# diaoenmao/HeteroFL-Computation-and-Communication-Efficient-Federated-Learning-for-Heterogeneous-Clients

Measured on AMD Instinct MI355X. Metric: local-train samples/sec/node, higher is better.
Workload: dtype bfloat16; 1 GPU; model=resnet18, dataset=CIFAR10, control_name=1_100_0.1_iid_fix_a1-e1_bn_1_1, active_clients=10, local_epochs=5, global_batch=10, parallelism=client-dp1, engine=batched

## Files before the change

### heterofl_amd/fed/batched.py

```python
import math

import numpy as np
import torch
import torch.nn as nn
import torch.nn.functional as F

from .. import ops as native_ops


class BConv2d(nn.Module):

    def __init__(self, R, in_ch, out_ch, kernel, stride, padding, bias):
        super().__init__()
        self.R, self.in_ch, self.out_ch = R, in_ch, out_ch
        self.stride, self.padding = stride, padding
        self.weight = nn.Parameter(torch.empty(R * out_ch, in_ch, kernel, kernel))
        nn.init.kaiming_uniform_(self.weight, a=math.sqrt(5))
        if bias:
            bound = 1 / math.sqrt(in_ch * kernel * kernel)
            self.bias = nn.Parameter(torch.empty(R * out_ch).uniform_(-bound, bound))
        else:
            self.bias = None

    def forward(self, x, residual=None):
        if native_ops.use_native(x) and native_ops.native_conv_enabled():
            from ..ops.fused import grouped_conv
            return grouped_conv(x, self.weight, self.bias, self.R,
                                self.stride, self.padding, residual=residual)
        y = F.conv2d(x, self.weight, self.bias, stride=self.stride,
                     padding=self.padding, groups=self.R)
        return y if residual is None else y + residual


class BBatchNorm2d(nn.Module):

    def __init__(self, R, ch):
        super().__init__()
        self.weight = nn.Parameter(torch.ones(R * ch))
        self.bias = nn.Parameter(torch.zeros(R * ch))

    def forward(self, x):
        return F.batch_norm(x, None, None, self.weight, self.bias,
                            training=True, eps=1e-5)


class BGroupNorm(nn.Module):

    def __init__(self, R, groups, ch):
        super().__init__()
        self.num_groups = R * groups
        self.weight = nn.Parameter(torch.ones(R * ch))
        self.bias = nn.Parameter(torch.zeros(R * ch))

    def forward(self, x):
        return F.group_norm(x, self.num_groups, self.weight, self.bias, eps=1e-5)


class BLinear(nn.Module):

    def __init__(self, R, in_f, out_f):
        super().__init__()
        self.weight = nn.Parameter(torch.empty(R, out_f, in_f))
        nn.init.kaiming_uniform_(self.weight, a=math.sqrt(5))
        self.bias = nn.Parameter(torch.zeros(R, out_f))

    def forward(self, x):
        return torch.einsum('nri,roi->nro', x, self.weight) + self.bias


def batched_norm(norm, R, ch):
    if norm == 'bn':
        return BBatchNorm2d(R, ch)
    if norm == 'in':
        return BGroupNorm(R, ch, ch)
    if norm == 'ln':
        return BGroupNorm(R, 1, ch)
    if norm == 'gn':
        return BGroupNorm(R, 4, ch)
    if norm == 'none':
        return nn.Identity()
    raise ValueError('Not valid norm')


class BNormReLU(nn.Module):

    def __init__(self, R, ch, norm, rate, scale):
        super().__init__()
        self.norm = norm
        self.rate = rate if scale else 1.0
        self.stats_sink = None
        if norm == 'in':
            self.groups = R * ch
        elif norm == 'ln':
            self.groups = R
        elif norm == 'gn':
            self.groups = R * 4
        else:
            self.groups = 0
        if norm != 'none':
            self.weight = nn.Parameter(torch.ones(R * ch))
            self.bias = nn.Parameter(torch.zeros(R * ch))

    def forward(self, x):
        if self.norm == 'none':
            if self.training and self.rate != 1.0:
                if native_ops.use_native(x):
                    from ..ops.fused import fused_scaler
                    x = fused_scaler(x, self.rate)
                else:
                    x = x / self.rate
            return F.relu(x)
        kind = 'bn' if self.norm == 'bn' else 'gn'
        if native_ops.use_native(x):
            if self.stats_sink is not None and kind == 'bn':
                ext = native_ops.require_native()
                y, mean, invstd = ext.bn_relu_fwd(x.contiguous(), self.weight,
                                                  self.bias, 1e-5)
                self.stats_sink(self, mean, invstd, x)
                return y
            from ..ops.fused import fused_norm_relu
            return fused_norm_relu(x, self.weight, self.bias, kind,
                                   self.groups)
        if self.stats_sink is not None and kind == 'bn':
            mean = x.mean(dim=(0, 2, 3))
            var = x.var(dim=(0, 2, 3), unbiased=False)
            self.stats_sink(self, mean, (var + 1e-5).rsqrt(), x)
        from ..ops.fused import eager_scaler_norm_relu
        r = self.rate if self.training else 1.0
        return eager_scaler_norm_relu(x, self.weight, self.bias, kind,
                                      self.groups, r)


class BMaxPool2(nn.Module):

    def forward(self, x):
        if native_ops.use_native(x):
            from ..ops.fused import fused_maxpool2
            return fused_maxpool2(x)
        return F.max_pool2d(x, 2)


class BScaler(nn.Module):
    def __init__(self, rate):
        super().__init__()
        self.rate = rate

    def forward(self, x):
        if not self.training or self.rate == 1.0:
            return x
        if native_ops.use_native(x):
            from ..ops.fused import fused_scaler
            return fused_scaler(x, self.rate)
        return x / self.rate


class BBlock(nn.Module):
    expansion = 1

    def __init__(self, R, in_planes, planes, stride, rate, norm, scale):
        super().__init__()
        self.n1 = BNormReLU(R, in_planes, norm, rate, scale)
        self.conv1 = BConv2d(R, in_planes, planes, 3, stride, 1, bias=False)
        self.n2 = BNormReLU(R, planes, norm, rate, scale)
        self.conv2 = BConv2d(R, planes, planes, 3, 1, 1, bias=False)
        if stride != 1 or in_planes != self.expansion * planes:
            self.shortcut = BConv2d(R, in_planes, self.expansion * planes,
                                    1, stride, 0, bias=False)

    def forward(self, x):
        out = self.n1(x)
        shortcut = self.shortcut(out) if hasattr(self, 'shortcut') else x
        out = self.conv1(out)
        return self.conv2(self.n2(out), residual=shortcut)


class BBottleneck(nn.Module):
    expansion = 4

    def __init__(self, R, in_planes, planes, stride, rate, norm, scale):
        super().__init__()
        self.n1 = BNormReLU(R, in_planes, norm, rate, scale)
        self.conv1 = BConv2d(R, in_planes, planes, 1, 1, 0, bias=False)
        self.n2 = BNormReLU(R, planes, norm, rate, scale)
        self.conv2 = BConv2d(R, planes, planes, 3, stride, 1, bias=False)
        self.n3 = BNormReLU(R, planes, norm, rate, scale)
        self.conv3 = BConv2d(R, planes, self.expansion * planes, 1, 1, 0,
                             bias=False)
        if stride != 1 or in_planes != self.expansion * planes:
            self.shortcut = BConv2d(R, in_planes, self.expansion * planes,
                                    1, stride, 0, bias=False)

    def forward(self, x):
        out = self.n1(x)
        shortcut = self.shortcut(out) if hasattr(self, 'shortcut') else x
        out = self.conv1(out)
        out = self.conv2(self.n2(out))
        return self.conv3(self.n3(out), residual=shortcut)


class BatchedResNet(nn.Module):

    def __init__(self, R, data_shape, hidden_size, num_blocks, num_classes,
                 rate, norm, scale, block=BBlock):
        super().__init__()
        self.R = R
        self.num_classes = num_classes
        self.data_ch = data_shape[0]
        self.in_planes = hidden_size[0]
        self.conv1 = BConv2d(R, data_shape[0], hidden_size[0], 3, 1, 1, bias=False)
        self.layer1 = self._make_layer(R, block, hidden_size[0], num_blocks[0], 1, rate, norm, scale)
        self.layer2 = self._make_layer(R, block, hidden_size[1], num_blocks[1], 2, rate, norm, scale)
        self.layer3 = self._make_layer(R, block, hidden_size[2], num_blocks[2], 2, rate, norm, scale)
        self.layer4 = self._make_layer(R, block, hidden_size[3], num_blocks[3], 2, rate, norm, scale)
        self.n4 = BNormReLU(R, hidden_size[3] * block.expansion, norm, rate, scale)
        self.linear = BLinear(R, hidden_size[3] * block.expansion, num_classes)

    def _make_layer(self, R, block, planes, num_blocks, stride, rate, norm, scale):
        strides = [stride] + [1] * (num_blocks - 1)
        layers = []
        for s in strides:
            layers.append(block(R, self.in_planes, planes, s, rate, norm, scale))
            self.in_planes = planes * block.expansion
        return nn.Sequential(*layers)

    def forward(self, x):
        out = self.conv1(x)
        out = self.layer1(out)
        out = self.layer2(out)
        out = self.layer3(out)
        out = self.layer4(out)
        out = self.n4(out)
        if native_ops.use_native(out):
            from ..ops.fused import fused_head
            return fused_head(out, self.linear.weight, self.linear.bias,
                              self.R)
        out = F.adaptive_avg_pool2d(out, 1)
        out = out.view(out.size(0), self.R, -1)
        return self.linear(out)


class BatchedConv(nn.Module):

    def __init__(self, R, data_shape, hidden_size, num_classes, rate, norm, scale):
        super().__init__()
        self.R = R
        self.num_classes = num_classes
        blocks = []
        in_ch = data_shape[0]
        for i, out_ch in enumerate(hidden_size):
            blocks.append(BConv2d(R, in_ch, out_ch, 3, 1, 1, bias=True))
            blocks.append(nn.Identity())
            blocks.append(BNormReLU(R, out_ch, norm, rate, scale))
            blocks.append(nn.Identity())
            if i != len(hidden_size) - 1:
                blocks.append(BMaxPool2())
            in_ch = out_ch
        self.blocks = nn.Sequential(*blocks)
        self._feat = hidden_size[-1]
        self.head = BLinear(R, hidden_size[-1], num_classes)

    def forward(self, x):
        out = self.blocks(x)
        if native_ops.use_native(out):
            from ..ops.fused import fused_head
            return fused_head(out, self.head.weight, self.head.bias, self.R)
        out = F.adaptive_avg_pool2d(out, 1).view(out.size(0), self.R, -1)
        return self.head(out)


def pack_states(batched, locals_list):
    R = batched.R
    bsd = batched.state_dict()
    key_map = _key_map(batched, locals_list[0])
    with torch.no_grad():
        for bk, lk in key_map.items():
            bt = bsd[bk]
            vals = [locals_list[r][lk] for r in range(R)]
            if bt.dim() == 3:
                src = torch.stack(vals, 0)
            elif bt.dim() == 2:
                src = torch.stack(vals, 0)
            else:
                src = torch.cat(vals, 0)
            bt.copy_(src.to(bt.device, bt.dtype))


def unpack_states(batched, template_keys):
    R = batched.R
    bsd = batched.state_dict()
    key_map = _key_map_from_keys(batched, template_keys)
    outs = [dict() for _ in range(R)]
    for bk, lk in key_map.items():
        bt = bsd[bk].detach()
        if bt.dim() in (2, 3):
            for r in range(R):
                outs[r][lk] = bt[r].clone()
        else:
            per = bt.size(0) // R
            for r in range(R):
                outs[r][lk] = bt[r * per:(r + 1) * per].clone()
    return outs


def _key_map(batched, local_sd):
    return _key_map_from_keys(batched, list(local_sd.keys()))


def _key_map_from_keys(batched, local_keys):
    bkeys = list(batched.state_dict().keys())
    if isinstance(batched, BatchedConv):
        lin_w = [k for k in local_keys if 'weight' in k][-1]
        lin_b = [k for k in local_keys if 'bias' in k][-1]
        m = {}
        for bk in bkeys:
            if bk == 'head.weight':
                m[bk] = lin_w
            elif bk == 'head.bias':
                m[bk] = lin_b
            else:
                m[bk] = bk
        return m
    return {bk: bk for bk in bkeys}


def batched_masked_ce(scores, labels, label_masks, metrics=None):
    if native_ops.use_native(scores):
        from ..ops.fused import fused_masked_ce
        return fused_masked_ce(scores, labels, label_masks, metrics)
    N, R, C = scores.shape
    if label_masks is not None:
        scores = scores.masked_fill(label_masks.unsqueeze(0) == 0, 0)
    logp = F.log_softmax(scores, dim=2)
    nll = -logp.gather(2, labels.unsqueeze(2)).squeeze(2)
    losses = nll.mean(0)
    if metrics is not None:
        with torch.no_grad():
            correct = (scores.argmax(2) == labels).float().sum(0)
            metrics[:, 0] += losses.detach() * N
            metrics[:, 1] += correct
            metrics[:, 2] += N
    return losses


def per_client_clip_(params, R, max_norm=1.0):
    sq = None
    views = []
    for p in params:
        if p.grad is None:
            continue
        g = p.grad
        if g.size(0) % R != 0:
            raise RuntimeError(f'grad shape {tuple(g.shape)} not divisible by R={R}')
        v = g.view(R, -1)
        views.append((g, v))
        s = (v.float() ** 2).sum(dim=1)
        sq = s if sq is None else sq + s
    if sq is None:
        return None
    total = sq.sqrt()
    scale = (max_norm / (total + 1e-6)).clamp(max=1.0)
    for g, v in views:
        v.mul_(scale.unsqueeze(1).to(v.dtype))
    return total


class DeviceAugment:

    def __init__(self, data_name, device):
        self.data_name = data_name
        if data_name in ('MNIST', 'FashionMNIST'):
            mean, std = (0.1307,), (0.3081,)
            self.crop = False
        else:
            mean, std = (0.4914, 0.4822, 0.4465), (0.2023, 0.1994, 0.2010)
            self.crop = True
        self.mean = torch.tensor(mean, device=device).view(1, -1, 1, 1)
        self.std = torch.tensor(std, device=device).view(1, -1, 1, 1)

    def __call__(self, img_u8, train=True):
        x = img_u8.permute(0, 3, 1, 2).float().div_(255.0)
        n, C, H, W = x.shape
        if train and self.crop:
            pad = 4
            xp = F.pad(x, [pad] * 4)
            dy = torch.randint(0, 2 * pad + 1, (n,), device=x.device)
            dx = torch.randint(0, 2 * pad + 1, (n,), device=x.device)
            rows = dy.view(n, 1) + torch.arange(H, device=x.device).view(1, H)
            idx_r = rows.view(n, 1, H, 1).expand(n, C, H, W + 2 * pad)
            xp = xp.gather(2, idx_r)
            cols = dx.view(n, 1) + torch.arange(W, device=x.device).view(1, W)
            idx_c = cols.view(n, 1, 1, W).expand(n, C, H, W)
            x = xp.gather(3, idx_c)
            flip = torch.rand(n, device=x.device) < 0.5
            x = torch.where(flip.view(n, 1, 1, 1), x.flip(-1), x)
        return (x - self.mean) / self.std


class BatchedClientTrainer:

    def __init__(self, cfg):
        self.cfg = cfg
        self.device = torch.device(cfg['device'])
        self.dataset = None
        self.data_split = None
        self.augment = None
        self._amp = (cfg.get('compute_dtype') in ('bfloat16', 'fp8')
                     and self.device.type == 'cuda')
        if self.device.type == 'cuda':
            native_ops.set_fp8(cfg.get('compute_dtype') == 'fp8')
        self._shard_cache = {}
        self._model_cache = {}
        self._graph_cache = {}

    def set_data(self, dataset, data_split):
        self.dataset = dataset['train']
        self.data_split = data_split['train']
        self.augment = DeviceAugment(self.cfg['data_name'], self.device)
        self._shard_cache.clear()

    def _shard(self, user):
        if user not in self._shard_cache:
            idx = torch.tensor(self.data_split[user], dtype=torch.long)
            img = self.dataset.img[idx]
            if img.dim() == 3:
                img = img.unsqueeze(-1)
            labels = torch.tensor([self.dataset.target[i] for i in idx.tolist()],
                                  dtype=torch.long)
            self._shard_cache[user] = (img.to(self.device, non_blocking=True),
                                       labels.to(self.device, non_blocking=True))
        return self._shard_cache[user]

    def _batched_model(self, rate, R, scaler_rate=None):
        key = (rate, R) if scaler_rate is None else (rate, R, scaler_rate)
        if key not in self._model_cache:
            cfg = self.cfg
            name = cfg['model_name']
            if scaler_rate is None:
                scaler_rate = rate / cfg['global_model_rate']
            if 'resnet' in name:
                hidden = [int(np.ceil(rate * h)) for h in cfg['resnet']['hidden_size']]
                nb, blk = {'resnet18': ([2, 2, 2, 2], BBlock),
                           'resnet34': ([3, 4, 6, 3], BBlock),
                           'resnet50': ([3, 4, 6, 3], BBottleneck),
                           'resnet101': ([3, 4, 23, 3], BBottleneck),
                           'resnet152': ([3, 8, 36, 3], BBottleneck)}[name]
                model = BatchedResNet(R, cfg['data_shape'], hidden, nb,
                                      cfg['classes_size'], scaler_rate,
                                      cfg['norm'], cfg['scale'], block=blk)
            elif name == 'conv':
                hidden = [int(np.ceil(rate * h)) for h in cfg['conv']['hidden_size']]
                model = BatchedConv(R, cfg['data_shape'], hidden,
                                    cfg['classes_size'], scaler_rate,
                                    cfg['norm'], cfg['scale'])
            else:
                raise NotImplementedError(name)
            self._model_cache[key] = model.to(self.device)
        return self._model_cache[key]

    def train_clients(self, client_slots, user_idx, local_parameters,
                      model_rate, make_loader, label_split, lr, logger=None):
        if self.dataset is None:
            raise RuntimeError('BatchedClientTrainer.set_data was not called')
        cfg = self.cfg
        B = cfg['batch_size']['train']
        groups = {}
        for m in client_slots:
            u = user_idx[m]
            n = len(self.data_split[u])
            sched = tuple([B] * (n // B) + ([n % B] if n % B else []))
            groups.setdefault((model_rate[u], sched), []).append(m)
        out = []
        import os as _os
        gsplit = int(_os.environ.get('HETEROFL_GROUP_SPLIT', '1'))
        split_groups = {}
        for (rate, sched), slots in groups.items():
            if gsplit > 1 and self.device.type == 'cuda' \
                    and len(slots) >= 2 * gsplit:
                per = (len(slots) + gsplit - 1) // gsplit
                for si in range(0, len(slots), per):
                    split_groups[(rate, sched, si)] = slots[si:si + per]
            else:
                split_groups[(rate, sched, 0)] = slots
        graphed = []
        for (rate, sched, tag), slots in split_groups.items():
            use_graph = (self.device.type == 'cuda'
                         and cfg.get('hip_graphs', True)
                         and len(set(sched)) == 1)
            if use_graph:
                graphed.append((rate, sched, slots, tag))
            else:
                out.extend(self._train_group(rate, sched, slots, user_idx,
                                             local_parameters, label_split,
                                             lr, logger))
        if graphed:
            preps = [self._prepare_graphed(rate, sched, slots, user_idx,
                                           [local_parameters[m]
                                            for m in slots],
                                           label_split, lr, tag)
                     for rate, sched, slots, tag in graphed]
            from .runner import _phase_timer
            with _phase_timer('2d.replay'):
                if len(preps) > 1:
                    if not hasattr(self, '_streams') or \
                            len(self._streams) < len(preps):
                        self._streams = [torch.cuda.Stream()
                                         for _ in range(len(preps))]
                    cur = torch.cuda.current_stream()
                    events = []
                    for (gs, x_cat, y_cat, nspe), st in zip(preps,
                                                            self._streams):
                        st.wait_stream(cur)
                        with torch.cuda.stream(st):
                            gs.run_epochs(x_cat, y_cat, nspe)
                        ev = torch.cuda.Event()
                        ev.record(st)
                        events.append(ev)
                    for ev in events:
                        cur.wait_event(ev)
                else:
                    gs, x_cat, y_cat, nspe = preps[0]
                    gs.run_epochs(x_cat, y_cat, nspe)
            for (rate, sched, slots, tag), (gs, _, _, _) in zip(graphed,
                                                                preps):
                out.extend(self._finish_graphed(
                    gs, slots, [local_parameters[m] for m in slots], logger))
        return out

    def _graph_step(self, rate, sched, R, lr, tag=0):
        from .graphs import GraphedGroupStep
        key = (rate, R, tuple(sched), lr, tag)
        if key not in self._graph_cache:
            cfg = self.cfg
            model = self._batched_model(rate, R)
            self._model_cache.pop((rate, R), None)
            model.train(True)
            capacity = sum(sched) * cfg['num_epochs']['local']
            self._graph_cache[key] = GraphedGroupStep(
                model, R, sched[0], lr, cfg['momentum'], cfg['weight_decay'],
                cfg['classes_size'], capacity, self._amp, self.device)
        return self._graph_cache[key]

    def _train_group(self, rate, sched, slots, user_idx, local_parameters,
                     label_split, lr, logger=None):
        cfg = self.cfg
        R = len(slots)
        device = self.device
        use_graph = (device.type == 'cuda' and cfg.get('hip_graphs', True)
                     and len(set(sched)) == 1)
        locals_list = [local_parameters[m] for m in slots]
        if use_graph:
            return self._train_group_graphed(rate, sched, slots, user_idx,
                                             locals_list, label_split, lr,
                                             logger)
        model = self._batched_model(rate, R)
        pack_states(model, locals_list)
        model.train(True)
        params = [p for p in model.parameters() if p.requires_grad]
        native = native_ops.use_native(device)
        if native:
            if not hasattr(self, '_opt_cache'):
                self._opt_cache = {}
            cached = self._opt_cache.get((rate, R))
            if cached is None or cached[0] is not model:
                from ..ops.fused import FusedClipSGD
                for p in params:
                    p.grad = torch.zeros_like(p)
                bufs = [torch.zeros_like(p) for p in params]
                cached = (model, FusedClipSGD(params,
                                              [p.grad for p in params],
                                              bufs, R, device))
                self._opt_cache[(rate, R)] = cached
            fopt = cached[1]
            for b in fopt.bufs:
                b.zero_()
            opt = None
        else:
            opt = torch.optim.SGD(params, lr=lr, momentum=cfg['momentum'],
                                  weight_decay=cfg['weight_decay'])
        masks = None
        if cfg['mask']:
            masks = torch.zeros(R, cfg['classes_size'], device=device)
            for i, m in enumerate(slots):
                masks[i, label_split[user_idx[m]]] = 1
        shards = [self._shard(user_idx[m]) for m in slots]
        n = sum(sched)
        for _ in range(cfg['num_epochs']['local']):
            xs, ys = [], []
            for img, lab in shards:
                perm = torch.randperm(img.size(0), device=device)
                xs.append(self.augment(img[perm], train=True))
                ys.append(lab[perm])
            x_all = torch.stack(xs, 1)
            x_all = x_all.reshape(n, -1, x_all.size(-2), x_all.size(-1))
            if self._amp:
                x_all = x_all.to(torch.bfloat16)
            y_all = torch.stack(ys, 1)
            off = 0
            for bs in sched:
                xb = x_all[off:off + bs]
                yb = y_all[off:off + bs]
                off += bs
                if native:
                    torch._foreach_zero_([p.grad for p in params])
                else:
                    opt.zero_grad(set_to_none=True)
                with torch.autocast('cuda', torch.bfloat16, enabled=self._amp):
                    scores = model(xb)
                losses = batched_masked_ce(scores.float(), yb, masks)
                losses.sum().backward()
                if native:
                    fopt.step(1.0, lr, cfg['momentum'], cfg['weight_decay'])
                else:
                    per_client_clip_(params, R, 1.0)
                    opt.step()
                if logger is not None:
                    with torch.no_grad():
                        sc = scores
                        if masks is not None:
                            sc = sc.masked_fill(masks.unsqueeze(0) == 0, 0)
                        pred = sc.argmax(dim=2)
                        acc = (pred == yb).float().mean(0) * 100.0
                        for i in range(R):
                            logger.append({'Local-Loss': losses[i].item(),
                                           'Local-Accuracy': acc[i].item()},
                                          'train', n=bs)
        template_keys = list(locals_list[0].keys())
        states = unpack_states(model, template_keys)
        cpu_or_dev = [{k: v for k, v in st.items()} for st in states]
        return list(zip(slots, cpu_or_dev))

    def _prepare_graphed(self, rate, sched, slots, user_idx, locals_list,
                         label_split, lr, tag=0):
        from .runner import _phase_timer
        cfg = self.cfg
        R = len(slots)
        device = self.device
        with _phase_timer('2a.graph_build'):
            gs = self._graph_step(rate, sched, R, lr, tag)
            if gs.graph is None:
                gs.ensure_captured()
        with _phase_timer('2b.pack'):
            pack_states(gs.model, locals_list)
        masks = None
        if cfg['mask']:
            masks = torch.zeros(R, cfg['classes_size'], device=device)
            for i, m in enumerate(slots):
                masks[i, label_split[user_idx[m]]] = 1
        gs.begin_round(masks)
        shards = [self._shard(user_idx[m]) for m in slots]
        n = sum(sched)
        E = cfg['num_epochs']['local']
        with _phase_timer('2c.stage_augment'):
            xs_ep, ys_ep = [], []
            for _ in range(E):
                xs, ys = [], []
                for img, lab in shards:
                    perm = torch.randperm(img.size(0), device=device)
                    xs.append(self.augment(img[perm], train=True))
                    ys.append(lab[perm])
                x_all = torch.stack(xs, 1)
                xs_ep.append(x_all.reshape(n, -1, x_all.size(-2), x_all.size(-1)))
                ys_ep.append(torch.stack(ys, 1))
            x_cat = torch.cat(xs_ep, 0)
            if self._amp:
                x_cat = x_cat.to(torch.bfloat16)
            y_cat = torch.cat(ys_ep, 0)
        return gs, x_cat, y_cat, len(sched)

    def _finish_graphed(self, gs, slots, locals_list, logger=None):
        from .runner import _phase_timer
        R = len(slots)
        if logger is not None:
            m = gs.metrics.detach().cpu()
            for i in range(R):
                cnt = max(int(m[i, 2].item()), 1)
                logger.append({'Local-Loss': m[i, 0].item() / cnt,
                               'Local-Accuracy': m[i, 1].item() / cnt * 100.0},
                              'train', n=cnt)
        with _phase_timer('2e.unpack'):
            template_keys = list(locals_list[0].keys())
            states = unpack_states(gs.model, template_keys)
        return list(zip(slots, [dict(st) for st in states]))
```

### heterofl_amd/fed/graphs.py

```python
import torch

from .. import ops as native_ops
from .batched import batched_masked_ce


class GraphedGroupStep:

    def __init__(self, model, R, batch, lr, momentum, weight_decay, classes,
                 capacity, amp, device):
        self.model = model
        self.R = R
        self.batch = batch
        self.lr = lr
        self.momentum = momentum
        self.weight_decay = weight_decay
        self.amp = amp
        self.device = device
        self.params = [p for p in model.parameters() if p.requires_grad]
        self.bufs = [torch.zeros_like(p) for p in self.params]
        self.capacity = capacity
        shape = self._input_shape()
        xdt = torch.bfloat16 if amp else torch.float32
        self.x_all = torch.zeros(capacity, *shape, device=device, dtype=xdt)
        self.y_all = torch.zeros(capacity, R, dtype=torch.long, device=device)
        self.masks = torch.ones(R, classes, device=device)
        self.counter = torch.zeros(1, dtype=torch.long, device=device)
        self.metrics = torch.zeros(R, 3, device=device)
        self.graph = None
        self._arange = torch.arange(batch, device=device)
        self._native = (device.type == 'cuda' and native_ops.use_native(device))
        self._capturing = False
        self._captured_grads = None
        self._shadows = False
        if self._native:
            native_ops.require_native()
            from ..ops.fused import GraphClipSGD
            self.opt = GraphClipSGD(self.params, self.bufs, R, device)

    def _input_shape(self):
        m = self.model
        w = next(p for p in m.parameters() if p.dim() == 4)
        in_ch = w.size(1)
        hw = 32 if in_ch == 3 else 28
        return (self.R * in_ch, hw, hw)

    def _one_step(self):
        idx = self.counter * self.batch + self._arange
        xb = self.x_all.index_select(0, idx)
        yb = self.y_all.index_select(0, idx)
        if self._native:
            with torch.autocast('cuda', torch.bfloat16, enabled=self.amp):
                scores = self.model(xb)
            losses = batched_masked_ce(scores.float(), yb, self.masks,
                                       metrics=self.metrics)
            raw = torch.autograd.grad(losses.sum(), self.params)
            grads = [t if t.is_contiguous() else t.contiguous() for t in raw]
            self._captured_grads = grads
            if not self._capturing:
                self.opt.bind(grads)
            self.opt.launch(1.0, self.lr, self.momentum, self.weight_decay)
            with torch.no_grad():
                self.counter += 1
            return
        with torch.autocast('cuda', torch.bfloat16, enabled=self.amp):
            scores = self.model(xb)
            losses = batched_masked_ce(scores.float(), yb, self.masks)
        loss = losses.sum()
        raw = torch.autograd.grad(loss, self.params)
        with torch.no_grad():
            grads = [g.contiguous() for g in raw]
            sq = None
            views = [g.view(self.R, -1) for g in grads]
            for v in views:
                s = (v.float() ** 2).sum(dim=1)
                sq = s if sq is None else sq + s
            scale = (1.0 / (sq.sqrt() + 1e-6)).clamp(max=1.0)
            for v in views:
                v.mul_(scale.unsqueeze(1).to(v.dtype))
            torch._foreach_add_(grads, self.params, alpha=self.weight_decay)
            torch._foreach_mul_(self.bufs, self.momentum)
            torch._foreach_add_(self.bufs, grads)
            torch._foreach_add_(self.params, self.bufs, alpha=-self.lr)
            pred = scores.argmax(dim=2)
            correct = (pred == yb).float().sum(0)
            self.metrics[:, 0] += losses.detach() * self.batch
            self.metrics[:, 1] += correct
            self.metrics[:, 2] += self.batch
            self.counter += 1

    def capture(self):
        saved_p = [p.detach().clone() for p in self.params]
        saved_b = [b.clone() for b in self.bufs]
        saved_m = self.metrics.clone()
        torch.cuda.synchronize()
        s = torch.cuda.Stream()
        s.wait_stream(torch.cuda.current_stream())
        with torch.cuda.stream(s):
            for _ in range(3):
                self.counter.zero_()
                self._one_step()
        torch.cuda.current_stream().wait_stream(s)
        self.counter.zero_()
        self.graph = torch.cuda.CUDAGraph()
        self._capturing = True
        with torch.cuda.graph(self.graph):
            self._one_step()
        self._capturing = False
        if self._native:
            self.opt.bind(self._captured_grads)
        with torch.no_grad():
            for p, sp in zip(self.params, saved_p):
                p.copy_(sp)
            for b, sb in zip(self.bufs, saved_b):
                b.copy_(sb)
            self.metrics.copy_(saved_m)
            self.counter.zero_()
        if self._shadows:
            from .batched_lm import refresh_shadows
            refresh_shadows(self.model)
        torch.cuda.synchronize()

    def begin_round(self, masks):
        with torch.no_grad():
            if masks is not None:
                self.masks.copy_(masks)
            else:
                self.masks.fill_(1)
            for b in self.bufs:
                b.zero_()
            self.metrics.zero_()

    def run_epochs(self, x_epochs, y_epochs, steps_per_epoch):
        total = x_epochs.size(0)
        with torch.no_grad():
            self.x_all[:total].copy_(x_epochs)
            self.y_all[:total].copy_(y_epochs)
            self.counter.zero_()
        n_steps = total // self.batch
        if self.graph is None:
            self.capture()
        for _ in range(n_steps):
            self.graph.replay()

    def ensure_captured(self):
        if self.graph is None:
            self.capture()


class LMGraphedStep:

    def __init__(self, model, R, n_rows, bptt, n_win, lr, momentum,
                 weight_decay, num_tokens, amp, device):
        self.model = model
        self.R = R
        self.bptt = bptt
        self.n_win = n_win
        self.lr = lr
        self.momentum = momentum
        self.weight_decay = weight_decay
        self.amp = amp
        self.device = device
        self.params = [p for p in model.parameters() if p.requires_grad]
        self.bufs = [torch.zeros_like(p) for p in self.params]
        self.windows = torch.zeros(n_win, R, n_rows, bptt, dtype=torch.long,
                                   device=device)
        self.masks = torch.ones(R, num_tokens, device=device)
        self.counter = torch.zeros(1, dtype=torch.long, device=device)
        self.metrics = torch.zeros(R, 3, device=device)
        self.graph = None
        self._capturing = False
        self._captured_grads = None
        self._native = (device.type == 'cuda' and native_ops.use_native(device))
        smap = getattr(model, '_shadow_map', None) or {}
        self._shadows = bool(smap)
        if self._native:
            from ..ops.fused import GraphClipSGD
            self.opt = GraphClipSGD(self.params, self.bufs, R, device,
                                    shadows=[smap.get(id(p))
                                             for p in self.params]
                                    if smap else None)

    def _one_step(self):
        w = self.counter - (self.counter // self.n_win) * self.n_win
        tokens = self.windows.index_select(0, w).squeeze(0)
        self._step_on(tokens)
        with torch.no_grad():
            self.counter += 1

    def tail_step(self, tokens):
        self._step_on(tokens)
        if self._native and self.graph is not None:
            self.opt.bind(self._graph_grads)

    def _step_on(self, tokens):
        from .batched_lm import lm_masked_ce
        with torch.autocast('cuda', torch.bfloat16,
                            enabled=self.amp and not self._shadows):
            logits = self.model(tokens)
        losses = lm_masked_ce(logits, tokens, self.masks)
        with torch.no_grad():
            n = tokens.size(1)
            ld = losses.detach()
            self.metrics[:, 0] += ld * n
            self.metrics[:, 1] += torch.exp(ld.clamp(max=30.0)) * n
            self.metrics[:, 2] += n
        if self._native:
            raw = torch.autograd.grad(losses.sum(), self.params)
            grads = [t if t.is_contiguous() else t.contiguous() for t in raw]
            self._captured_grads = grads
            if not self._capturing:
                self.opt.bind(grads)
            self.opt.launch(1.0, self.lr, self.momentum, self.weight_decay)
            if self._shadows:
                from ..ops.fused import bump_rng
                bump_rng(self.device)
        else:
            raw = torch.autograd.grad(losses.sum(), self.params)
            with torch.no_grad():
                grads = [g.contiguous() for g in raw]
                sq = None
                views = [g.view(self.R, -1) for g in grads]
                for v in views:
                    s = (v.float() ** 2).sum(dim=1)
                    sq = s if sq is None else sq + s
                scale = (1.0 / (sq.sqrt() + 1e-6)).clamp(max=1.0)
                for v in views:
                    v.mul_(scale.unsqueeze(1).to(v.dtype))
                torch._foreach_add_(grads, self.params,
                                    alpha=self.weight_decay)
                torch._foreach_mul_(self.bufs, self.momentum)
                torch._foreach_add_(self.bufs, grads)
                torch._foreach_add_(self.params, self.bufs, alpha=-self.lr)

    def capture(self):
        saved_p = [p.detach().clone() for p in self.params]
        saved_b = [b.clone() for b in self.bufs]
        saved_m = self.metrics.clone()
        torch.cuda.synchronize()
        s = torch.cuda.Stream()
        s.wait_stream(torch.cuda.current_stream())
        with torch.cuda.stream(s):
            for _ in range(3):
                self.counter.zero_()
                self._one_step()
        torch.cuda.current_stream().wait_stream(s)
        self.counter.zero_()
        self.graph = torch.cuda.CUDAGraph()
        self._capturing = True
        with torch.cuda.graph(self.graph):
            self._one_step()
        self._capturing = False
        if self._native:
            self._graph_grads = self._captured_grads
            self.opt.bind(self._graph_grads)
        with torch.no_grad():
            for p, sp in zip(self.params, saved_p):
                p.copy_(sp)
            for b, sb in zip(self.bufs, saved_b):
                b.copy_(sb)
            self.metrics.copy_(saved_m)
            self.counter.zero_()
        if self._shadows:
            from .batched_lm import refresh_shadows
            refresh_shadows(self.model)
        torch.cuda.synchronize()

    def begin_round(self, rows, masks):
        with torch.no_grad():
            for w in range(self.n_win):
                self.windows[w].copy_(
                    rows[:, :, w * self.bptt:(w + 1) * self.bptt])
            if masks is not None:
                self.masks.copy_(masks)
            else:
                self.masks.fill_(1)
            for b in self.bufs:
                b.zero_()
            self.metrics.zero_()
            self.counter.zero_()

    def run_window_pass(self):
        if self.graph is None:
            self.capture()
        for _ in range(self.n_win):
            self.graph.replay()
```

### heterofl_amd/ops/__init__.py

```python
import os

import torch

_ext = None
_ext_err = None


def _load():
    global _ext, _ext_err
    if _ext is not None or _ext_err is not None:
        return _ext
    try:
        from . import _heterofl_hip as ext
        _ext = ext
    except ImportError as e:
        _ext_err = e
    return _ext


def native_available():
    return _load() is not None


def require_native():
    if os.environ.get('HETEROFL_FORCE_EAGER') == '1':
        return None
    ext = _load()
    if ext is None:
        raise RuntimeError(
            f'heterofl_amd native HIP extension is not built '
            f'(import error: {_ext_err}). Build it with '
            f'`python setup.py build_ext --inplace` (PYTORCH_ROCM_ARCH=gfx950).')
    return ext


def use_native(tensor_or_device=None):
    if os.environ.get('HETEROFL_FORCE_EAGER') == '1':
        return False
    if isinstance(tensor_or_device, torch.Tensor):
        is_cuda = tensor_or_device.is_cuda
    elif tensor_or_device is not None:
        is_cuda = torch.device(tensor_or_device).type == 'cuda'
    else:
        is_cuda = torch.cuda.is_available()
    return is_cuda


def native_conv_enabled():
    return os.environ.get('HETEROFL_NATIVE_CONV', '1') == '1'


_FP8 = False


def set_fp8(on):
    global _FP8
    _FP8 = bool(on)


def fp8_enabled():
    return _FP8


_LARGE_CONV = os.environ.get('HETEROFL_LARGE_CONV', '0') == '1'


def set_large_conv(on):
    global _LARGE_CONV
    prev = _LARGE_CONV
    _LARGE_CONV = bool(on)
    return prev


def large_conv_enabled():
    return _LARGE_CONV
```

### heterofl_amd/ops/csrc/bindings.cpp

```cpp
#include <torch/extension.h>

std::vector<at::Tensor> bn_relu_fwd(at::Tensor x, at::Tensor gamma,
                                    at::Tensor beta, double eps);
std::vector<at::Tensor> bn_relu_bwd(at::Tensor dy, at::Tensor x,
                                    at::Tensor gamma, at::Tensor beta,
                                    at::Tensor mean, at::Tensor invstd);
std::string bn_relu_route(const std::string& direction, int64_t N, int64_t C,
                          int64_t HW, int64_t elem_size, bool aligned);
std::vector<at::Tensor> gn_relu_fwd(at::Tensor x, at::Tensor gamma,
                                    at::Tensor beta, int64_t G, double eps);
std::vector<at::Tensor> gn_relu_bwd(at::Tensor dy, at::Tensor x,
                                    at::Tensor gamma, at::Tensor beta,
                                    at::Tensor mean, at::Tensor invstd,
                                    int64_t G);
std::vector<at::Tensor> masked_ce_fwd(at::Tensor scores, at::Tensor labels,
                                      at::Tensor mask, at::Tensor metrics);
at::Tensor masked_ce_bwd(at::Tensor scores, at::Tensor labels, at::Tensor mask,
                         at::Tensor up);
std::vector<at::Tensor> build_chunk_table(std::vector<at::Tensor> grads,
                                          std::vector<at::Tensor> params,
                                          std::vector<at::Tensor> bufs,
                                          int64_t R, int64_t chunk_elems,
                                          std::vector<at::Tensor> shadows);
void fill_chunk_table(at::Tensor blob, std::vector<at::Tensor> grads,
                      std::vector<at::Tensor> params,
                      std::vector<at::Tensor> bufs, int64_t R,
                      int64_t chunk_elems, std::vector<at::Tensor> shadows);
void clip_sgd_step(at::Tensor table_blob, int64_t n_chunks,
                   at::Tensor chunk_client, at::Tensor partials,
                   at::Tensor normsq, double max_norm, double lr,
                   double momentum, double weight_decay);
at::Tensor conv_fwd(at::Tensor x, at::Tensor w, at::Tensor bias,
                    at::Tensor residual, int64_t groups, int64_t stride,
                    int64_t pad, int64_t fp8);
at::Tensor conv_bwd_data(at::Tensor dy, at::Tensor w, int64_t groups,
                         int64_t stride, int64_t pad, int64_t H, int64_t W,
                         int64_t fp8);
at::Tensor conv_bwd_weight(at::Tensor dy, at::Tensor x, int64_t groups,
                           int64_t stride, int64_t pad, int64_t khw,
                           int64_t fp8);
std::tuple<std::string, int64_t, int64_t> conv_plan(
    const std::string& direction, int64_t G, int64_t N, int64_t Cin,
    int64_t H, int64_t W, int64_t Cout, int64_t khw, int64_t stride,
    int64_t pad, int64_t elem_size, int64_t fp8);
std::string conv_plan_variant(
    const std::string& direction, int64_t G, int64_t N, int64_t Cin,
    int64_t H, int64_t W, int64_t Cout, int64_t khw, int64_t stride,
    int64_t pad, int64_t elem_size, int64_t fp8);
at::Tensor mfma_probe(at::Tensor A, at::Tensor B);
std::vector<at::Tensor> head_fwd(at::Tensor feat, at::Tensor w, at::Tensor b,
                                 int64_t R);
std::vector<at::Tensor> attn_fwd(at::Tensor q, at::Tensor k, at::Tensor v,
                                 double temperature);
std::vector<at::Tensor> attn_bwd(at::Tensor dout, at::Tensor q, at::Tensor k,
                                 at::Tensor v, at::Tensor p,
                                 double temperature);
std::vector<at::Tensor> attn_fwd_block(at::Tensor q, at::Tensor k,
                                       at::Tensor v, double temperature);
std::vector<at::Tensor> attn_bwd_block(at::Tensor dout, at::Tensor q,
                                       at::Tensor k, at::Tensor v,
                                       at::Tensor out, at::Tensor lse,
                                       double temperature);
std::vector<at::Tensor> ln_fwd(at::Tensor x, at::Tensor gamma,
                               at::Tensor beta, int64_t R, double eps);
std::vector<at::Tensor> ln_bwd(at::Tensor dy, at::Tensor x, at::Tensor gamma,
                               at::Tensor mean, at::Tensor invstd, int64_t R);
std::vector<at::Tensor> lm_ce_fwd(at::Tensor logits, at::Tensor labels,
                                  at::Tensor mask, int64_t R);
at::Tensor lm_ce_bwd(at::Tensor logits, at::Tensor labels, at::Tensor mask,
                     at::Tensor row_max, at::Tensor row_logsum,
                     at::Tensor up, int64_t R);
std::vector<at::Tensor> head_bwd(at::Tensor dscores, at::Tensor pooled,
                                 at::Tensor w, int64_t R, int64_t H,
                                 int64_t W, bool bf16_feat, bool want_db);
void rng_bump(at::Tensor seed);
std::vector<at::Tensor> gelu_drop_fwd(at::Tensor x, at::Tensor seed,
                                      int64_t salt, double rate, double p);
at::Tensor gelu_drop_bwd(at::Tensor dy, at::Tensor x, at::Tensor mask,
                         double rate, double p);
std::vector<at::Tensor> res_drop_fwd(at::Tensor src, at::Tensor h,
                                     at::Tensor seed, int64_t salt,
                                     double rate, double p);
at::Tensor drop_scale_bwd(at::Tensor dt, at::Tensor mask, double rate,
                          double p);
at::Tensor token_mask(at::Tensor tokens, at::Tensor seed, int64_t salt,
                      double rate, int64_t mask_id);
at::Tensor embed_pos_fwd(at::Tensor ids, at::Tensor table, at::Tensor pos,
                         double rate);
std::vector<at::Tensor> embed_pos_bwd(at::Tensor dy, at::Tensor ids,
                                      int64_t V, int64_t P, double rate);
std::vector<at::Tensor> maxpool2_fwd(at::Tensor x);
void pack_slices(at::Tensor blob, int64_t n, int64_t max_rows);
void pack_slices_roll(at::Tensor spans, int64_t n_spans, at::Tensor blocks);
void combine_accumulate(at::Tensor table, int64_t n_tensors,
                        int64_t n_entries, at::Tensor blocks);
at::Tensor maxpool2_bwd(at::Tensor dy, at::Tensor arg, int64_t H,
                        int64_t W);
at::Tensor conv_pack_weight(at::Tensor w);
at::Tensor conv_fwd_large(at::Tensor x, at::Tensor packed, at::Tensor bias,
                          at::Tensor residual, int64_t stride, int64_t pad,
                          int64_t Cin, int64_t Cout, int64_t k);
at::Tensor bn_relu_infer(at::Tensor x, at::Tensor scale, at::Tensor shift);
std::vector<at::Tensor> eval_metrics(at::Tensor scores, at::Tensor labels,
                                     at::Tensor user_ptr,
                                     at::Tensor user_samples,
                                     at::Tensor label_mask);
at::Tensor lm_head_pack(at::Tensor w);
std::vector<at::Tensor> lm_head_ce(at::Tensor x, at::Tensor packed,
                                   at::Tensor bias, at::Tensor labels,
                                   at::Tensor vocab_mask, int64_t V,
                                   int64_t E, int64_t splits);
std::vector<at::Tensor> lm_head_topk(at::Tensor x, at::Tensor packed,
                                     at::Tensor bias, at::Tensor labels,
                                     at::Tensor vocab_mask, int64_t V,
                                     int64_t E, int64_t k, int64_t splits);
int64_t lm_head_topk_splits(int64_t M, int64_t V);

PYBIND11_MODULE(TORCH_EXTENSION_NAME, m) {
    m.def("bn_relu_fwd", &bn_relu_fwd, "fused sBN+ReLU forward");
    m.def("bn_relu_bwd", &bn_relu_bwd, "fused sBN+ReLU backward");
    m.def("bn_relu_route", &bn_relu_route,
          "name of the kernel route bn_relu_fwd / bn_relu_bwd would take; "
          "launches nothing");
    m.def("gn_relu_fwd", &gn_relu_fwd, "fused GroupNorm+ReLU forward");
    m.def("gn_relu_bwd", &gn_relu_bwd, "fused GroupNorm+ReLU backward");
    m.def("masked_ce_fwd", &masked_ce_fwd, "batched masked CE forward");
    m.def("masked_ce_bwd", &masked_ce_bwd, "batched masked CE backward");
    m.def("build_chunk_table", &build_chunk_table,
          "build clip+SGD chunk table");
    m.def("clip_sgd_step", &clip_sgd_step, "fused per-client clip+SGD step");
    m.def("fill_chunk_table", &fill_chunk_table,
          "fill a preallocated chunk table post-capture");
    m.def("conv_fwd", &conv_fwd, "MFMA implicit-GEMM grouped conv forward");
    m.def("conv_bwd_data", &conv_bwd_data, "MFMA grouped conv backward-data");
    m.def("conv_bwd_weight", &conv_bwd_weight,
          "MFMA grouped conv backward-weight (fp32 out)");
    m.def("conv_plan", &conv_plan,
          "(route, split, dynamic LDS bytes) the conv launchers would take; "
          "launches nothing");
    m.def("conv_plan_variant", &conv_plan_variant,
          "name of the kernel the conv launcher would launch; launches "
          "nothing");
    m.def("mfma_probe", &mfma_probe, "16x16x32 bf16 MFMA layout probe");
    m.def("head_fwd", &head_fwd, "fused avgpool+per-client-linear forward");
    m.def("head_bwd", &head_bwd, "fused head backward");
    m.def("attn_fwd", &attn_fwd, "fused small-S attention forward");
    m.def("attn_bwd", &attn_bwd, "fused small-S attention backward");
    m.def("attn_fwd_block", &attn_fwd_block,
          "blockwise (flash-style) attention forward, any S");
    m.def("attn_bwd_block", &attn_bwd_block,
          "blockwise attention backward (deterministic two-pass)");
    m.def("ln_fwd", &ln_fwd, "fused per-client LayerNorm forward");
    m.def("ln_bwd", &ln_bwd, "fused per-client LayerNorm backward");
    m.def("lm_ce_fwd", &lm_ce_fwd, "fused vocab-masked LM CE forward");
    m.def("lm_ce_bwd", &lm_ce_bwd, "fused vocab-masked LM CE backward");
    m.def("rng_bump", &rng_bump, "advance the device RNG seed cell");
    m.def("gelu_drop_fwd", &gelu_drop_fwd, "fused scaler+GELU+dropout fwd");
    m.def("gelu_drop_bwd", &gelu_drop_bwd, "fused scaler+GELU+dropout bwd");
    m.def("res_drop_fwd", &res_drop_fwd,
          "fused scaler+dropout+residual-add fwd");
    m.def("drop_scale_bwd", &drop_scale_bwd,
          "dropout-mask * 1/rate backward");
    m.def("token_mask", &token_mask, "Bernoulli token masking (in-kernel RNG)");
    m.def("embed_pos_fwd", &embed_pos_fwd,
          "fused token+positional embedding gather with Scaler");
    m.def("embed_pos_bwd", &embed_pos_bwd,
          "deterministic embedding backward (fp32 master grads)");
    m.def("maxpool2_fwd", &maxpool2_fwd, "2x2/2 MaxPool forward (saves argmax)");
    m.def("pack_slices", &pack_slices,
          "one-launch distribute slice pack from a descriptor table");
    m.def("pack_slices_roll", &pack_slices_roll,
          "one-launch distribute pack of periodic-window (rolled / per-head) "
          "slices");
    m.def("combine_accumulate", &combine_accumulate,
          "one-launch deterministic combine accumulator + count (gather "
          "form)");
    m.def("maxpool2_bwd", &maxpool2_bwd, "2x2/2 MaxPool backward");
    m.def("conv_pack_weight", &conv_pack_weight,
          "one-time tap-major bf16 repack for conv_fwd_large");
    m.def("conv_fwd_large", &conv_fwd_large,
          "large-batch forward conv (bf16, groups=1, packed weight)");
    m.def("bn_relu_infer", &bn_relu_infer,
          "eval-mode BN+ReLU from folded scale/shift");
    m.def("eval_metrics", &eval_metrics,
          "per-user Local + Global evaluation sums (deterministic)");
    m.def("lm_head_pack", &lm_head_pack,
          "one-time padded bf16 repack of the LM vocabulary head");
    m.def("lm_head_ce", &lm_head_ce,
          "fused vocabulary projection + cross-entropy (no logits written)");
    m.def("lm_head_topk", &lm_head_topk,
          "fused vocabulary projection + top-k + log-sum-exp (no logits "
          "written)");
    m.def("lm_head_topk_splits", &lm_head_topk_splits,
          "lm_head_topk's own choice of splits for M rows");
}
```

### heterofl_amd/ops/csrc/fused_norm.hip

```cpp
#include "common.h"

template <typename T, bool STAGE>
__global__ void __launch_bounds__(256)
bn_relu_fwd_kernel(const T* __restrict__ x, const float* __restrict__ gamma,
                   const float* __restrict__ beta, T* __restrict__ y,
                   float* __restrict__ mean_out, float* __restrict__ invstd_out,
                   int N, int C, int HW, float eps) {
    const int c = blockIdx.x;
    __shared__ float scratch[2 * 256 / WAVE];
    extern __shared__ __attribute__((aligned(16))) char smem[];
    T* stage = (T*)smem;
    float s1 = 0.f, s2 = 0.f;
    const long chan_off = (long)c * HW;
    const long samp_stride = (long)C * HW;
    for (int i = threadIdx.x; i < N * HW; i += blockDim.x) {
        const int n = i / HW, hw = i - n * HW;
        const T raw = x[n * samp_stride + chan_off + hw];
        if (STAGE) stage[i] = raw;
        const float v = (float)raw;
        s1 += v;
        s2 += v * v;
    }
    block_reduce2(s1, s2, scratch);
    const float inv_m = 1.f / (N * HW);
    const float mean = s1 * inv_m;
    const float var = fmaxf(s2 * inv_m - mean * mean, 0.f);
    const float invstd = rsqrtf(var + eps);
    if (threadIdx.x == 0) {
        mean_out[c] = mean;
        invstd_out[c] = invstd;
    }
    const float g = gamma ? gamma[c] : 1.f;
    const float b = beta ? beta[c] : 0.f;
    const float scale = invstd * g;
    const float shift = b - mean * scale;
    for (int i = threadIdx.x; i < N * HW; i += blockDim.x) {
        const int n = i / HW, hw = i - n * HW;
        const long off = n * samp_stride + chan_off + hw;
        const float v = STAGE ? (float)stage[i] : ld_f32(x + off);
        st_f32(y + off, fmaxf(v * scale + shift, 0.f));
    }
}

template <typename T>
__global__ void __launch_bounds__(256)
bn_sums_kernel(const T* __restrict__ x, float* __restrict__ partials, int N,
               int C, int HW, int S) {
    const int c = blockIdx.x;
    const int s = blockIdx.y;
    const int chunk = (N + S - 1) / S;
    const int n1 = min(N, (s + 1) * chunk);
    const long chan_off = (long)c * HW;
    const long samp_stride = (long)C * HW;
    float s1 = 0.f, s2 = 0.f;
    for (int n = s * chunk; n < n1; ++n) {
        const T* base = x + n * samp_stride + chan_off;
        for (int hw = threadIdx.x; hw < HW; hw += blockDim.x) {
            const float v = ld_f32(base + hw);
            s1 += v;
            s2 += v * v;
        }
    }
    __shared__ float scratch[2 * 256 / WAVE];
    block_reduce2(s1, s2, scratch);
    if (threadIdx.x == 0) {
        partials[((long)c * S + s) * 2] = s1;
        partials[((long)c * S + s) * 2 + 1] = s2;
    }
}

__global__ void __launch_bounds__(256)
bn_finalize_kernel(const float* __restrict__ partials,
                   const float* __restrict__ gamma,
                   const float* __restrict__ beta,
                   float* __restrict__ mean_out,
                   float* __restrict__ invstd_out,
                   float* __restrict__ scale_shift, int C, int S,
                   float inv_m, float eps) {
    const int c = blockIdx.x * blockDim.x + threadIdx.x;
    if (c >= C) return;
    float s1 = 0.f, s2 = 0.f;
    for (int s = 0; s < S; ++s) {
        s1 += partials[((long)c * S + s) * 2];
        s2 += partials[((long)c * S + s) * 2 + 1];
    }
    const float mean = s1 * inv_m;
    const float var = fmaxf(s2 * inv_m - mean * mean, 0.f);
    const float invstd = rsqrtf(var + eps);
    mean_out[c] = mean;
    invstd_out[c] = invstd;
    const float g = gamma ? gamma[c] : 1.f;
    const float b = beta ? beta[c] : 0.f;
    const float scale = invstd * g;
    scale_shift[2 * c] = scale;
    scale_shift[2 * c + 1] = b - mean * scale;
}

template <typename T>
__global__ void __launch_bounds__(256)
bn_apply_relu_kernel(const T* __restrict__ x,
                     const float* __restrict__ scale_shift,
                     T* __restrict__ y, int N, int C, int HW, int S) {
    const int c = blockIdx.x;
    const int s = blockIdx.y;
    const int chunk = (N + S - 1) / S;
    const int n1 = min(N, (s + 1) * chunk);
    const long chan_off = (long)c * HW;
    const long samp_stride = (long)C * HW;
    const float scale = scale_shift[2 * c];
    const float shift = scale_shift[2 * c + 1];
    for (int n = s * chunk; n < n1; ++n) {
        const long off = n * samp_stride + chan_off;
        for (int hw = threadIdx.x; hw < HW; hw += blockDim.x)
            st_f32(y + off + hw, fmaxf(ld_f32(x + off + hw) * scale + shift,
                                       0.f));
    }
}

template <typename T, bool STAGE>
__global__ void __launch_bounds__(256)
bn_relu_bwd_kernel(const T* __restrict__ dy, const T* __restrict__ x,
                   const float* __restrict__ gamma, const float* __restrict__ beta,
                   const float* __restrict__ mean, const float* __restrict__ invstd,
                   T* __restrict__ dx, float* __restrict__ dgamma,
                   float* __restrict__ dbeta, int N, int C, int HW) {
    const int c = blockIdx.x;
    __shared__ float scratch[2 * 256 / WAVE];
    extern __shared__ __attribute__((aligned(16))) char smem[];
    T* sx = (T*)smem;
    T* sd = sx + (STAGE ? N * HW : 0);
    const long chan_off = (long)c * HW;
    const long samp_stride = (long)C * HW;
    const float m = mean[c], is = invstd[c];
    const float g = gamma ? gamma[c] : 1.f;
    const float b = beta ? beta[c] : 0.f;
    float s1 = 0.f, s2 = 0.f;
    for (int i = threadIdx.x; i < N * HW; i += blockDim.x) {
        const int n = i / HW, hw = i - n * HW;
        const long off = n * samp_stride + chan_off + hw;
        const T xr = x[off];
        const float xh = ((float)xr - m) * is;
        const float pre = xh * g + b;
        const float d = pre > 0.f ? ld_f32(dy + off) : 0.f;
        if (STAGE) {
            sx[i] = xr;
            sd[i] = (T)d;
        }
        s1 += d;
        s2 += d * xh;
    }
    block_reduce2(s1, s2, scratch);
    if (threadIdx.x == 0) {
        dbeta[c] = s1;
        dgamma[c] = s2;
    }
    const float inv_M = 1.f / (N * HW);
    const float k1 = s1 * inv_M, k2 = s2 * inv_M;
    const float gis = g * is;
    for (int i = threadIdx.x; i < N * HW; i += blockDim.x) {
        const int n = i / HW, hw = i - n * HW;
        const long off = n * samp_stride + chan_off + hw;
        float xh, d;
        if (STAGE) {
            xh = ((float)sx[i] - m) * is;
            d = (float)sd[i];
        } else {
            xh = (ld_f32(x + off) - m) * is;
            const float pre = xh * g + b;
            d = pre > 0.f ? ld_f32(dy + off) : 0.f;
        }
        st_f32(dx + off, gis * (d - k1 - xh * k2));
    }
}

constexpr int BN_VEC_U = 4;

struct RowWalk {
    int n, j, dn, dj, vpr;
    __device__ __forceinline__ RowWalk(int v, int vpr_) : vpr(vpr_) {
        n = v / vpr;
        j = v - n * vpr;
        dn = 256 / vpr;
        dj = 256 - dn * vpr;
    }
    __device__ __forceinline__ void step() {
        j += dj;
        n += dn;
        if (j >= vpr) {
            j -= vpr;
            ++n;
        }
    }
};

template <typename T>
__global__ void __launch_bounds__(256)
bn_relu_fwd_vec_kernel(const T* __restrict__ x,
                       const float* __restrict__ gamma,
                       const float* __restrict__ beta, T* __restrict__ y,
                       float* __restrict__ mean_out,
                       float* __restrict__ invstd_out, int N, int C, int HW,
                       float eps) {
    constexpr int V = 16 / sizeof(T);
    const int c = blockIdx.x;
    __shared__ float scratch[2 * 256 / WAVE];
    extern __shared__ __attribute__((aligned(16))) char smem[];
    const T* stage = (const T*)smem;
    uint4* stage4 = (uint4*)smem;
    const int M = N * HW;
    const int nvec = M / V;
    const long samp_stride = (long)C * HW;
    const T* xc = x + (long)c * HW;
    T* yc = y + (long)c * HW;
    RowWalk rw(threadIdx.x, HW / V);
    for (int v0 = threadIdx.x; v0 < nvec; v0 += 256 * BN_VEC_U) {
        uint4 r[BN_VEC_U];
        const long off0 = rw.n * samp_stride + rw.j * V;
#pragma unroll
        for (int u = 0; u < BN_VEC_U; ++u) {
            const long off = v0 + u * 256 < nvec
                                 ? rw.n * samp_stride + rw.j * V : off0;
            r[u] = *(const uint4*)(xc + off);
            rw.step();
        }
#pragma unroll
        for (int u = 0; u < BN_VEC_U; ++u)
            if (v0 + u * 256 < nvec) stage4[v0 + u * 256] = r[u];
    }
    __syncthreads();
    float s1 = 0.f, s2 = 0.f;
#pragma unroll 8
    for (int i = threadIdx.x; i < M; i += 256) {
        const float v = (float)stage[i];
        s1 += v;
        s2 += v * v;
    }
    block_reduce2(s1, s2, scratch);
    const float inv_m = 1.f / (N * HW);
    const float mean = s1 * inv_m;
    const float var = fmaxf(s2 * inv_m - mean * mean, 0.f);
    const float invstd = rsqrtf(var + eps);
    if (threadIdx.x == 0) {
        mean_out[c] = mean;
        invstd_out[c] = invstd;
    }
    const float g = gamma ? gamma[c] : 1.f;
    const float b = beta ? beta[c] : 0.f;
    const float scale = invstd * g;
    const float shift = b - mean * scale;
    RowWalk ww(threadIdx.x, HW / V);
    for (int v = threadIdx.x; v < nvec; v += 256) {
        float f[V];
        unpack16<T>(stage4[v], f);
#pragma unroll
        for (int e = 0; e < V; ++e) f[e] = fmaxf(f[e] * scale + shift, 0.f);
        *(uint4*)(yc + ww.n * samp_stride + ww.j * V) = pack16<T>(f);
        ww.step();
    }
}

template <typename T>
__global__ void __launch_bounds__(256)
bn_relu_bwd_vec_kernel(const T* __restrict__ dy, const T* __restrict__ x,
                       const float* __restrict__ gamma,
                       const float* __restrict__ beta,
                       const float* __restrict__ mean,
                       const float* __restrict__ invstd, T* __restrict__ dx,
                       float* __restrict__ dgamma, float* __restrict__ dbeta,
                       int N, int C, int HW) {
    constexpr int V = 16 / sizeof(T);
    const int c = blockIdx.x;
    __shared__ float scratch[2 * 256 / WAVE];
    extern __shared__ __attribute__((aligned(16))) char smem[];
    const int M = N * HW;
    const int nvec = M / V;
    const T* sx = (const T*)smem;
    const T* sd = sx + M;
    uint4* sx4 = (uint4*)sx;
    uint4* sd4 = (uint4*)sd;
    const long samp_stride = (long)C * HW;
    const T* xc = x + (long)c * HW;
    const T* dyc = dy + (long)c * HW;
    T* dxc = dx + (long)c * HW;
    const float m = mean[c], is = invstd[c];
    const float g = gamma ? gamma[c] : 1.f;
    const float b = beta ? beta[c] : 0.f;
    RowWalk rw(threadIdx.x, HW / V);
    for (int v0 = threadIdx.x; v0 < nvec; v0 += 256 * BN_VEC_U) {
        uint4 rx[BN_VEC_U], rd[BN_VEC_U];
        const long off0 = rw.n * samp_stride + rw.j * V;
#pragma unroll
        for (int u = 0; u < BN_VEC_U; ++u) {
            const long off = v0 + u * 256 < nvec
                                 ? rw.n * samp_stride + rw.j * V : off0;
            rx[u] = *(const uint4*)(xc + off);
            rd[u] = *(const uint4*)(dyc + off);
            rw.step();
        }
#pragma unroll
        for (int u = 0; u < BN_VEC_U; ++u)
            if (v0 + u * 256 < nvec) {
                sx4[v0 + u * 256] = rx[u];
                sd4[v0 + u * 256] = rd[u];
            }
    }
    __syncthreads();
    float s1 = 0.f, s2 = 0.f;
#pragma unroll 8
    for (int i = threadIdx.x; i < M; i += 256) {
        const float xh = ((float)sx[i] - m) * is;
        const float pre = xh * g + b;
        const float d = pre > 0.f ? ld_f32(sd + i) : 0.f;
        s1 += d;
        s2 += d * xh;
    }
    block_reduce2(s1, s2, scratch);
    if (threadIdx.x == 0) {
        dbeta[c] = s1;
        dgamma[c] = s2;
    }
    const float inv_M = 1.f / (N * HW);
    const float k1 = s1 * inv_M, k2 = s2 * inv_M;
    const float gis = g * is;
    RowWalk ww(threadIdx.x, HW / V);
    for (int v = threadIdx.x; v < nvec; v += 256) {
        float fx[V], fd[V];
        unpack16<T>(sx4[v], fx);
        unpack16<T>(sd4[v], fd);
#pragma unroll
        for (int e = 0; e < V; ++e) {
            const float xh = (fx[e] - m) * is;
            const float pre = xh * g + b;
            const float d = pre > 0.f ? fd[e] : 0.f;
            fd[e] = gis * (d - k1 - xh * k2);
        }
        *(uint4*)(dxc + ww.n * samp_stride + ww.j * V) = pack16<T>(fd);
        ww.step();
    }
}

__device__ __forceinline__ float mul_rn(float a, float b) {
#pragma clang fp contract(off)
    return a * b;
}
__device__ __forceinline__ float sub_rn(float a, float b) {
#pragma clang fp contract(off)
    return a - b;
}

template <typename T, bool STAGE>
__global__ void __launch_bounds__(256)
gn_relu_fwd_kernel(const T* __restrict__ x, const float* __restrict__ gamma,
                   const float* __restrict__ beta, T* __restrict__ y,
                   float* __restrict__ mean_out, float* __restrict__ invstd_out,
                   int N, int C, int HW, int G, float eps) {
    const int ng = blockIdx.x;
    const int n = ng / G, j = ng - n * G;
    const int cpg = C / G;
    __shared__ float scratch[2 * 256 / WAVE];
    extern __shared__ __attribute__((aligned(16))) char smem[];
    T* stage = (T*)smem;
    const long base = (long)n * C * HW + (long)j * cpg * HW;
    const int M = cpg * HW;
    float s1 = 0.f, s2 = 0.f;
    for (int i = threadIdx.x; i < M; i += blockDim.x) {
        const T raw = x[base + i];
        if (STAGE) stage[i] = raw;
        const float v = (float)raw;
        s1 += v;
        s2 += v * v;
    }
    block_reduce2(s1, s2, scratch);
    const float inv_m = 1.f / M;
    const float mean = s1 * inv_m;
    const float var = fmaxf(sub_rn(mul_rn(s2, inv_m), mul_rn(mean, mean)),
                            0.f);
    const float invstd = rsqrtf(var + eps);
    if (threadIdx.x == 0) {
        mean_out[ng] = mean;
        invstd_out[ng] = invstd;
    }
    for (int i = threadIdx.x; i < M; i += blockDim.x) {
        const int c = j * cpg + i / HW;
        const float g = gamma ? gamma[c] : 1.f;
        const float b = beta ? beta[c] : 0.f;
        const float v = STAGE ? (float)stage[i] : ld_f32(x + base + i);
        st_f32(y + base + i, fmaxf((v - mean) * invstd * g + b, 0.f));
    }
}

template <typename T>
__global__ void __launch_bounds__(256)
gn_relu_bwd_kernel(const T* __restrict__ dy, const T* __restrict__ x,
                   const float* __restrict__ gamma, const float* __restrict__ beta,
                   const float* __restrict__ mean, const float* __restrict__ invstd,
                   T* __restrict__ dx, float* __restrict__ pgamma,
                   float* __restrict__ pbeta, int N, int C, int HW, int G) {
    const int ng = blockIdx.x;
    const int n = ng / G, j = ng - n * G;
    const int cpg = C / G;
    __shared__ float scratch[2 * 256 / WAVE];
    const long base = (long)n * C * HW + (long)j * cpg * HW;
    const int M = cpg * HW;
    const float m = mean[ng], is = invstd[ng];
    if (pgamma) {
        for (int cc = threadIdx.x; cc < cpg; cc += blockDim.x) {
            const int c = j * cpg + cc;
            const float g = gamma ? gamma[c] : 1.f;
            const float b = beta ? beta[c] : 0.f;
            float sg = 0.f, sb = 0.f;
            for (int hw = 0; hw < HW; ++hw) {
                const long off = base + (long)cc * HW + hw;
                const float xh = (ld_f32(x + off) - m) * is;
                const float pre = xh * g + b;
                const float d = pre > 0.f ? ld_f32(dy + off) : 0.f;
                sg += d * xh;
                sb += d;
            }
            pgamma[(long)n * C + c] = sg;
            pbeta[(long)n * C + c] = sb;
        }
    }
    float s1 = 0.f, s2 = 0.f;
    for (int i = threadIdx.x; i < M; i += blockDim.x) {
        const int c = j * cpg + i / HW;
        const float g = gamma ? gamma[c] : 1.f;
        const float b = beta ? beta[c] : 0.f;
        const float xh = (ld_f32(x + base + i) - m) * is;
        const float pre = xh * g + b;
        const float d = pre > 0.f ? ld_f32(dy + base + i) : 0.f;
        const float dg = mul_rn(d, g);
        s1 += dg;
        s2 += dg * xh;
    }
    block_reduce2(s1, s2, scratch);
    const float inv_M = 1.f / M;
    const float k1 = s1 * inv_M, k2 = s2 * inv_M;
    for (int i = threadIdx.x; i < M; i += blockDim.x) {
        const int c = j * cpg + i / HW;
        const float g = gamma ? gamma[c] : 1.f;
        const float b = beta ? beta[c] : 0.f;
        const float xh = (ld_f32(x + base + i) - m) * is;
        const float pre = xh * g + b;
        const float d = pre > 0.f ? ld_f32(dy + base + i) : 0.f;
        st_f32(dx + base + i,
               is * (sub_rn(mul_rn(d, g), k1) - xh * k2));
    }
}

#include <torch/extension.h>
#include <ATen/hip/HIPContext.h>

#define DISPATCH_FT(t, ...)                                                   \
    if ((t) == at::kFloat) { using scalar_t = float; __VA_ARGS__; }           \
    else if ((t) == at::kBFloat16) { using scalar_t = __hip_bfloat16; __VA_ARGS__; } \
    else { TORCH_CHECK(false, "unsupported dtype"); }

enum BnRoute { BN_VEC, BN_STAGED, BN_DIRECT, BN_SPLIT3 };

static BnRoute bn_route(bool bwd, long N, long HW, int esz, bool aligned) {
    const long M = N * HW;
    if (!bwd && M > 64 * 1024) return BN_SPLIT3;
    if ((bwd ? 2 : 1) * M * esz > 64 * 1024) return BN_DIRECT;
    if (stream_vec_on() && aligned && (HW * esz) % 16 == 0) return BN_VEC;
    return BN_STAGED;
}

std::string bn_relu_route(const std::string& direction, int64_t N, int64_t C,
                          int64_t HW, int64_t elem_size, bool aligned) {
    TORCH_CHECK(direction == "fwd" || direction == "bwd",
                "direction must be fwd or bwd");
    (void)C;
    static const char* names[] = {"vec", "staged", "direct", "split3"};
    return names[bn_route(direction == "bwd", N, HW, (int)elem_size,
                          aligned)];
}

std::vector<at::Tensor> bn_relu_fwd(at::Tensor x, at::Tensor gamma,
                                    at::Tensor beta, double eps) {
    TORCH_CHECK(x.is_cuda() && x.is_contiguous());
    const int N = x.size(0), C = x.size(1);
    const int HW = x.numel() / (N * C);
    auto y = at::empty_like(x);
    auto opts = x.options().dtype(at::kFloat);
    auto mean = at::empty({C}, opts);
    auto invstd = at::empty({C}, opts);
    auto stream = at::hip::getCurrentHIPStream();
    const long stage_bytes = (long)N * HW * x.element_size();
    const long M = (long)N * HW;
    if (M > 64 * 1024) {
        const int S = std::max(1, std::min(N, (4096 + C - 1) / C));
        auto partials = at::empty({(long)C * S * 2}, opts);
        auto scale_shift = at::empty({2L * C}, opts);
        DISPATCH_FT(x.scalar_type(), {
            hipLaunchKernelGGL(bn_sums_kernel<scalar_t>, dim3(C, S),
                               dim3(256), 0, stream,
                               (const scalar_t*)x.data_ptr(),
                               partials.data_ptr<float>(), N, C, HW, S);
            hipLaunchKernelGGL(bn_finalize_kernel,
                               dim3((C + 255) / 256), dim3(256), 0, stream,
                               partials.data_ptr<float>(),
                               gamma.defined() ? gamma.data_ptr<float>()
                                               : nullptr,
                               beta.defined() ? beta.data_ptr<float>()
                                              : nullptr,
                               mean.data_ptr<float>(),
                               invstd.data_ptr<float>(),
                               scale_shift.data_ptr<float>(), C, S,
                               (float)(1.0 / M), (float)eps);
            hipLaunchKernelGGL(bn_apply_relu_kernel<scalar_t>, dim3(C, S),
                               dim3(256), 0, stream,
                               (const scalar_t*)x.data_ptr(),
                               scale_shift.data_ptr<float>(),
                               (scalar_t*)y.data_ptr(), N, C, HW, S);
        });
        return {y, mean, invstd};
    }
    const BnRoute route = bn_route(false, N, HW, (int)x.element_size(),
                                   ptr_aligned(x.data_ptr(), 16) &&
                                       ptr_aligned(y.data_ptr(), 16));
    const float* gp = gamma.defined() ? gamma.data_ptr<float>() : nullptr;
    const float* bp = beta.defined() ? beta.data_ptr<float>() : nullptr;
    DISPATCH_FT(x.scalar_type(), {
        auto kern = route == BN_VEC ? bn_relu_fwd_vec_kernel<scalar_t>
                    : route == BN_STAGED ? bn_relu_fwd_kernel<scalar_t, true>
                                         : bn_relu_fwd_kernel<scalar_t, false>;
        hipLaunchKernelGGL(kern, dim3(C), dim3(256),
                           route == BN_DIRECT ? 0 : (int)stage_bytes, stream,
                           (const scalar_t*)x.data_ptr(), gp, bp,
                           (scalar_t*)y.data_ptr(), mean.data_ptr<float>(),
                           invstd.data_ptr<float>(), N, C, HW, (float)eps);
    });
    return {y, mean, invstd};
}

std::vector<at::Tensor> bn_relu_bwd(at::Tensor dy, at::Tensor x,
                                    at::Tensor gamma, at::Tensor beta,
                                    at::Tensor mean, at::Tensor invstd) {
    const int N = x.size(0), C = x.size(1);
    const int HW = x.numel() / (N * C);
    auto dx = at::empty_like(x);
    auto opts = x.options().dtype(at::kFloat);
    auto dgamma = at::empty({C}, opts);
    auto dbeta = at::empty({C}, opts);
    auto dyc = dy.contiguous();
    auto stream = at::hip::getCurrentHIPStream();
    const long stage_bytes = 2L * N * (x.numel() / (N * C)) * x.element_size();
    const BnRoute route = bn_route(true, N, HW, (int)x.element_size(),
                                   ptr_aligned(x.data_ptr(), 16) &&
                                       ptr_aligned(dyc.data_ptr(), 16) &&
                                       ptr_aligned(dx.data_ptr(), 16));
    const float* gp = gamma.defined() ? gamma.data_ptr<float>() : nullptr;
    const float* bp = beta.defined() ? beta.data_ptr<float>() : nullptr;
    DISPATCH_FT(x.scalar_type(), {
        auto kern = route == BN_VEC ? bn_relu_bwd_vec_kernel<scalar_t>
                    : route == BN_STAGED ? bn_relu_bwd_kernel<scalar_t, true>
                                         : bn_relu_bwd_kernel<scalar_t, false>;
        hipLaunchKernelGGL(kern, dim3(C), dim3(256),
                           route == BN_DIRECT ? 0 : (int)stage_bytes, stream,
                           (const scalar_t*)dyc.data_ptr(),
                           (const scalar_t*)x.data_ptr(), gp, bp,
                           mean.data_ptr<float>(), invstd.data_ptr<float>(),
                           (scalar_t*)dx.data_ptr(), dgamma.data_ptr<float>(),
                           dbeta.data_ptr<float>(), N, C, HW);
    });
    return {dx, dgamma, dbeta};
}

std::vector<at::Tensor> gn_relu_fwd(at::Tensor x, at::Tensor gamma,
                                    at::Tensor beta, int64_t G, double eps) {
    TORCH_CHECK(x.is_cuda() && x.is_contiguous());
    const int N = x.size(0), C = x.size(1);
    const int HW = x.numel() / (N * C);
    TORCH_CHECK(C % G == 0, "channels not divisible by groups");
    auto y = at::empty_like(x);
    auto opts = x.options().dtype(at::kFloat);
    auto mean = at::empty({N * G}, opts);
    auto invstd = at::empty({N * G}, opts);
    auto stream = at::hip::getCurrentHIPStream();
    const long gsb = ((long)C / G) * (x.numel() / (N * C)) * x.element_size();
    DISPATCH_FT(x.scalar_type(), {
        if (gsb <= 64 * 1024)
            hipLaunchKernelGGL((gn_relu_fwd_kernel<scalar_t, true>),
                               dim3(N * G), dim3(256), (int)gsb, stream,
                               (const scalar_t*)x.data_ptr(),
                               gamma.defined() ? gamma.data_ptr<float>()
                                               : nullptr,
                               beta.defined() ? beta.data_ptr<float>()
                                              : nullptr,
                               (scalar_t*)y.data_ptr(), mean.data_ptr<float>(),
                               invstd.data_ptr<float>(), N, C, HW, (int)G,
                               (float)eps);
        else
            hipLaunchKernelGGL((gn_relu_fwd_kernel<scalar_t, false>),
                               dim3(N * G), dim3(256), 0, stream,
                               (const scalar_t*)x.data_ptr(),
                               gamma.defined() ? gamma.data_ptr<float>()
                                               : nullptr,
                               beta.defined() ? beta.data_ptr<float>()
                                              : nullptr,
                               (scalar_t*)y.data_ptr(), mean.data_ptr<float>(),
                               invstd.data_ptr<float>(), N, C, HW, (int)G,
                               (float)eps);
    });
    return {y, mean, invstd};
}

__global__ void __launch_bounds__(256)
gn_grad_reduce_kernel(const float* __restrict__ pgamma,
                      const float* __restrict__ pbeta,
                      float* __restrict__ dgamma, float* __restrict__ dbeta,
                      int N, int C) {
    const int c = blockIdx.x * blockDim.x + threadIdx.x;
    if (c >= C) return;
    float sg = 0.f, sb = 0.f;
    for (int n = 0; n < N; ++n) {
        sg += pgamma[(long)n * C + c];
        sb += pbeta[(long)n * C + c];
    }
    dgamma[c] = sg;
    dbeta[c] = sb;
}

std::vector<at::Tensor> gn_relu_bwd(at::Tensor dy, at::Tensor x,
                                    at::Tensor gamma, at::Tensor beta,
                                    at::Tensor mean, at::Tensor invstd,
                                    int64_t G) {
    const int N = x.size(0), C = x.size(1);
    const int HW = x.numel() / (N * C);
    auto dx = at::empty_like(x);
    auto opts = x.options().dtype(at::kFloat);
    auto pgamma = at::empty({N, C}, opts);
    auto pbeta = at::empty({N, C}, opts);
    auto dgamma = at::empty({C}, opts);
    auto dbeta = at::empty({C}, opts);
    auto dyc = dy.contiguous();
    auto stream = at::hip::getCurrentHIPStream();
    DISPATCH_FT(x.scalar_type(), {
        hipLaunchKernelGGL(gn_relu_bwd_kernel<scalar_t>, dim3(N * G), dim3(256),
                           0, stream,
                           (const scalar_t*)dyc.data_ptr(),
                           (const scalar_t*)x.data_ptr(),
                           gamma.defined() ? gamma.data_ptr<float>() : nullptr,
                           beta.defined() ? beta.data_ptr<float>() : nullptr,
                           mean.data_ptr<float>(), invstd.data_ptr<float>(),
                           (scalar_t*)dx.data_ptr(), pgamma.data_ptr<float>(),
                           pbeta.data_ptr<float>(), N, C, HW, (int)G);
    });
    hipLaunchKernelGGL(gn_grad_reduce_kernel, dim3((C + 255) / 256),
                       dim3(256), 0, stream, pgamma.data_ptr<float>(),
                       pbeta.data_ptr<float>(), dgamma.data_ptr<float>(),
                       dbeta.data_ptr<float>(), N, C);
    return {dx, dgamma, dbeta};
}
```

### heterofl_amd/ops/fused.py

```python
import torch
import torch.nn.functional as F

from . import require_native, use_native, large_conv_enabled


class _FusedNormReLU(torch.autograd.Function):

    @staticmethod
    def forward(ctx, x, weight, bias, kind, groups, eps):
        ext = require_native()
        x = x.contiguous()
        if kind == 'bn':
            y, mean, invstd = ext.bn_relu_fwd(x, weight, bias, eps)
        else:
            y, mean, invstd = ext.gn_relu_fwd(x, weight, bias, groups, eps)
        ctx.save_for_backward(x, weight, bias, mean, invstd)
        ctx.kind = kind
        ctx.groups = groups
        return y

    @staticmethod
    def backward(ctx, dy):
        ext = require_native()
        x, weight, bias, mean, invstd = ctx.saved_tensors
        if ctx.kind == 'bn':
            dx, dgamma, dbeta = ext.bn_relu_bwd(dy, x, weight, bias, mean,
                                                invstd)
        else:
            dx, dgamma, dbeta = ext.gn_relu_bwd(dy, x, weight, bias, mean,
                                                invstd, ctx.groups)
        return dx, dgamma, dbeta, None, None, None


def fused_norm_relu(x, weight, bias, kind, groups=1, eps=1e-5):
    return _FusedNormReLU.apply(x, weight, bias, kind, groups, eps)


def bn_relu_route(direction, N, C, HW, elem_size, aligned=True):
    ext = require_native()
    return ext.bn_relu_route(direction, N, C, HW, elem_size, aligned)


def eager_scaler_norm_relu(x, weight, bias, kind, groups, rate, eps=1e-5):
    if rate != 1.0:
        x = x / rate
    if kind == 'bn':
        x = F.batch_norm(x, None, None, weight, bias, training=True, eps=eps)
    else:
        x = F.group_norm(x, groups, weight, bias, eps=eps)
    return F.relu(x)


class _FusedMaskedCE(torch.autograd.Function):

    @staticmethod
    def forward(ctx, scores, labels, mask, metrics):
        ext = require_native()
        scores = scores.contiguous().float()
        (losses,) = ext.masked_ce_fwd(
            scores, labels.contiguous(),
            mask if mask is not None else torch.Tensor(),
            metrics if metrics is not None else torch.Tensor())
        ctx.save_for_backward(scores, labels,
                              mask if mask is not None else torch.Tensor())
        ctx.has_mask = mask is not None
        return losses

    @staticmethod
    def backward(ctx, up):
        ext = require_native()
        scores, labels, mask = ctx.saved_tensors
        dscores = ext.masked_ce_bwd(scores, labels,
                                    mask if ctx.has_mask else torch.Tensor(),
                                    up)
        return dscores, None, None, None


def fused_masked_ce(scores, labels, mask=None, metrics=None):
    return _FusedMaskedCE.apply(scores, labels, mask, metrics)


class FusedClipSGD:

    CHUNK = 65536

    def __init__(self, params, grads, bufs, R, device, shadows=None):
        ext = require_native()
        self.params = list(params)
        self.grads = list(grads)
        self.bufs = list(bufs)
        self.shadows = [s if s is not None else torch.Tensor()
                        for s in (shadows or [])]
        blob, n, clients = ext.build_chunk_table(
            self.grads, self.params, self.bufs, R, self.CHUNK, self.shadows)
        self.table = blob
        self.n_chunks = int(n.item())
        self.chunk_client = clients
        self.partials = torch.zeros(self.n_chunks, dtype=torch.float32,
                                    device=device)
        self.normsq = torch.zeros(R, dtype=torch.float32, device=device)

    def step(self, max_norm, lr, momentum, weight_decay):
        ext = require_native()
        ext.clip_sgd_step(self.table, self.n_chunks, self.chunk_client,
                          self.partials, self.normsq, max_norm, lr, momentum,
                          weight_decay)


class _GroupedConv(torch.autograd.Function):

    @staticmethod
    def forward(ctx, x, weight, bias, residual, groups, stride, pad):
        from . import fp8_enabled
        ext = require_native()
        fp8 = 1 if fp8_enabled() else 0
        x = x.contiguous()
        y = ext.conv_fwd(x, weight,
                         bias if bias is not None else torch.Tensor(),
                         residual.contiguous() if residual is not None
                         else torch.Tensor(),
                         groups, stride, pad, fp8)
        ctx.save_for_backward(x, weight)
        ctx.meta = (groups, stride, pad, bias is not None, fp8)
        return y

    @staticmethod
    def backward(ctx, dy):
        ext = require_native()
        x, w = ctx.saved_tensors
        groups, stride, pad, has_bias, fp8 = ctx.meta
        dy = dy.contiguous()
        dx = dw = db = None
        if ctx.needs_input_grad[0]:
            dx = ext.conv_bwd_data(dy, w, groups, stride, pad,
                                   x.size(2), x.size(3), fp8)
        if ctx.needs_input_grad[1]:
            dw = ext.conv_bwd_weight(dy, x, groups, stride, pad, w.size(2),
                                     fp8)
        if has_bias and ctx.needs_input_grad[2]:
            db = dy.float().sum(dim=(0, 2, 3))
        dres = dy if ctx.needs_input_grad[3] else None
        return dx, dw, db, dres, None, None, None


def grouped_conv(x, weight, bias, groups, stride, pad, residual=None):
    from . import fp8_enabled
    if large_conv_enabled() and groups == 1 and x.dtype == torch.bfloat16 \
            and not fp8_enabled() and not (torch.is_grad_enabled() and (
                x.requires_grad or weight.requires_grad
                or (bias is not None and bias.requires_grad)
                or (residual is not None and residual.requires_grad))) \
            and large_conv_route(x.size(0), weight.size(1), x.size(2),
                                 x.size(3), weight.size(0), weight.size(2),
                                 stride, pad):
        return conv_fwd_large(x, conv_pack_weight(weight.detach()),
                              None if bias is None else bias.detach(),
                              residual, stride, pad, weight.size(1),
                              weight.size(0), weight.size(2))
    return _GroupedConv.apply(x, weight, bias, residual, groups, stride, pad)


def conv_plan(direction, G, N, Cin, H, W, Cout, khw, stride, pad, elem_size,
              fp8):
    ext = require_native()
    return ext.conv_plan(direction, G, N, Cin, H, W, Cout, khw, stride, pad,
                         elem_size, fp8)


def conv_plan_variant(direction, G, N, Cin, H, W, Cout, khw, stride, pad,
                      elem_size, fp8):
    ext = require_native()
    return ext.conv_plan_variant(direction, G, N, Cin, H, W, Cout, khw,
                                 stride, pad, elem_size, fp8)


def large_conv_supported(k, stride, pad):
    return ((k == 3 and pad == 1) or (k == 1 and pad == 0)) \
        and stride in (1, 2)


def large_conv_route(N, Cin, H, W, Cout, k, stride, pad):
    if not large_conv_supported(k, stride, pad):
        return False
    OH = (H + 2 * pad - k) // stride + 1
    OW = (W + 2 * pad - k) // stride + 1
    P = N * OH * OW
    slabs = k * k * ((Cin + 31) // 32)
    old_us = 2.0 * P * (-(-Cout // 64) * 64) * Cin * k * k / 50e6
    cout_pad = 64 if Cout <= 64 else -(-Cout // 128) * 128
    large_us = max(15.0 + 1.2 * slabs,
                   2.0 * P * cout_pad * 32 * slabs / 150e6)
    return old_us > large_us


def conv_pack_weight(weight):
    ext = require_native()
    return ext.conv_pack_weight(weight.contiguous())


def conv_fwd_large(x, packed, bias, residual, stride, pad, Cin, Cout, k):
    ext = require_native()
    return ext.conv_fwd_large(
        x.contiguous(), packed,
        bias.float().contiguous() if bias is not None else torch.Tensor(),
        residual.contiguous() if residual is not None else torch.Tensor(),
        stride, pad, Cin, Cout, k)


def bn_relu_infer(x, scale, shift):
    if use_native(x):
        ext = require_native()
        return ext.bn_relu_infer(x.contiguous(), scale.float().contiguous(),
                                 shift.float().contiguous())
    shape = [1, -1] + [1] * (x.dim() - 2)
    y = x.float() * scale.view(shape) + shift.view(shape)
    return F.relu(y).to(x.dtype)


def fold_bn(weight, bias, mean, var, eps=1e-5):
    scale = weight.float() * torch.rsqrt(var.float() + eps)
    return scale, bias.float() - mean.float() * scale


def eval_metrics(scores, labels, user_ptr, user_samples, label_mask):
    scores = scores.float().contiguous()
    labels = labels.long().contiguous()
    user_ptr = user_ptr.long().contiguous()
    user_samples = user_samples.long().contiguous()
    label_mask = label_mask.float().contiguous()
    if use_native(scores):
        ext = require_native()
        local, glob = ext.eval_metrics(scores, labels, user_ptr, user_samples,
                                       label_mask)
        return local, glob
    U = user_ptr.numel() - 1
    C = scores.size(1)
    counts = user_ptr[1:] - user_ptr[:-1]
    owner = torch.repeat_interleave(torch.arange(U, device=scores.device),
                                    counts)

    def terms(sc, y):
        nll = F.cross_entropy(sc, y, reduction='none')
        mx = sc.max(dim=1, keepdim=True).values
        cls = torch.arange(C, device=sc.device).expand_as(sc)
        pred = torch.where(sc == mx, cls, torch.full_like(cls, C)).min(1).values
        return torch.stack([nll, (pred == y).float(),
                            torch.ones_like(nll)], 1)

    sc = scores[user_samples].masked_fill(label_mask[owner] == 0, 0)
    local = torch.zeros(U, 3, dtype=torch.float32, device=scores.device)
    if owner.numel():
        local.index_add_(0, owner, terms(sc, labels[user_samples]))
    glob = terms(scores, labels).sum(0) if scores.size(0) else \
        torch.zeros(3, device=scores.device)
    return local, glob


LM_HEAD_KPAD = 32
LM_HEAD_VPAD = 64


def lm_head_pack(weight, bias=None):
    V, E = weight.shape
    if bias is not None and tuple(bias.shape) != (V,):
        raise ValueError('lm_head_pack: bias must be (V,)')
    if not 1 <= E <= 256:
        raise ValueError('lm_head_pack: 1 <= E <= 256')
    if use_native(weight):
        ext = require_native()
        return ext.lm_head_pack(weight.detach().float().contiguous())
    Vp = -(-V // LM_HEAD_VPAD) * LM_HEAD_VPAD
    Ep = -(-E // LM_HEAD_KPAD) * LM_HEAD_KPAD
    out = torch.zeros(Vp, Ep, dtype=torch.float32, device=weight.device)
    out[:V, :E] = weight.detach().float()
    return out


def lm_head_ce(x, packed, bias, labels, vocab_mask, V, E, splits=0):
    if use_native(x):
        ext = require_native()
        none = torch.Tensor()
        nll, lse = ext.lm_head_ce(
            x.contiguous(), packed,
            bias.float().contiguous() if bias is not None else none,
            labels.long().contiguous(),
            vocab_mask.float().contiguous() if vocab_mask is not None
            else none, V, E, splits)
        return nll, lse
    logits = x.float() @ packed[:V, :E].float().t()
    if bias is not None:
        logits = logits + bias.float()
    if vocab_mask is not None:
        logits = logits.masked_fill(vocab_mask.view(1, V) == 0, 0)
    lse = torch.logsumexp(logits, dim=1)
    return lse - logits.gather(1, labels.long().view(-1, 1)).squeeze(1), lse


LM_HEAD_MAX_K = 8


def lm_head_topk(x, packed, bias, labels, vocab_mask, V, E, k, splits=0):
    if not 1 <= k <= min(LM_HEAD_MAX_K, V):
        raise ValueError('lm_head_topk: 1 <= k <= 8 and k <= V, got k={} '
                         'for V={}'.format(k, V))
    if use_native(x):
        ext = require_native()
        none = torch.Tensor()
        val, idx, lse, nll = ext.lm_head_topk(
            x.contiguous(), packed,
            bias.float().contiguous() if bias is not None else none,
            labels.long().contiguous() if labels is not None else none,
            vocab_mask.float().contiguous() if vocab_mask is not None
            else none, V, E, k, splits)
        return val, idx, lse, nll
    logits = x.float() @ packed[:V, :E].float().t()
    if bias is not None:
        logits = logits + bias.float()
    if vocab_mask is not None:
        logits = logits.masked_fill(vocab_mask.view(1, V) == 0, 0)
    lse = torch.logsumexp(logits, dim=1)
    nll = logits.new_empty(0)
    if labels is not None:
        nll = lse - logits.gather(1, labels.long().view(-1, 1)).squeeze(1)
    kth = torch.topk(logits, k, dim=1).values[:, -1:]
    keep = logits >= kth
    row, col = keep.nonzero(as_tuple=True)
    v = logits[row, col]
    o = torch.sort(v, descending=True, stable=True).indices
    o = o[torch.sort(row[o], stable=True).indices]
    first = keep.sum(1).cumsum(0) - keep.sum(1)
    pick = o[first.view(-1, 1) + torch.arange(k, device=x.device)]
    return v[pick], col[pick], lse, nll


def lm_head_route(M, E, V):
    return M >= 640 and V >= 33278 and E <= 256


class _FusedHead(torch.autograd.Function):

    @staticmethod
    def forward(ctx, feat, weight, bias, R):
        ext = require_native()
        feat = feat.contiguous()
        scores, pooled = ext.head_fwd(feat, weight,
                                      bias if bias is not None
                                      else torch.Tensor(), R)
        ctx.save_for_backward(pooled, weight)
        ctx.meta = (R, feat.size(2), feat.size(3),
                    feat.dtype == torch.bfloat16, bias is not None)
        return scores

    @staticmethod
    def backward(ctx, dscores):
        ext = require_native()
        pooled, weight = ctx.saved_tensors
        R, H, W, bf16_feat, has_bias = ctx.meta
        dw, db, dfeat = ext.head_bwd(dscores.contiguous().float(), pooled,
                                     weight, R, H, W, bf16_feat, has_bias)
        return dfeat, dw, (db if has_bias else None), None


def fused_head(feat, weight, bias, R):
    return _FusedHead.apply(feat, weight, bias, R)


class GraphClipSGD:

    CHUNK = 65536
    CHUNK_BYTES = 40

    def __init__(self, params, bufs, R, device, shadows=None):
        require_native()
        self.params = list(params)
        self.bufs = list(bufs)
        self.shadows = [s if s is not None else torch.Tensor()
                        for s in (shadows or [])]
        self.R = R
        clients = []
        for p in self.params:
            per = p.numel() // R
            nch = (per + self.CHUNK - 1) // self.CHUNK
            for r in range(R):
                clients.extend([r] * nch)
        self.n_chunks = len(clients)
        self.table = torch.zeros(self.n_chunks * self.CHUNK_BYTES,
                                 dtype=torch.uint8, device=device)
        self.chunk_client = torch.tensor(clients, dtype=torch.int32).to(device)
        self.partials = torch.zeros(self.n_chunks, dtype=torch.float32,
                                    device=device)
        self.normsq = torch.zeros(R, dtype=torch.float32, device=device)

    def bind(self, grads):
        ext = require_native()
        ext.fill_chunk_table(self.table, list(grads), self.params, self.bufs,
                             self.R, self.CHUNK, self.shadows)

    def launch(self, max_norm, lr, momentum, weight_decay):
        ext = require_native()
        ext.clip_sgd_step(self.table, self.n_chunks, self.chunk_client,
                          self.partials, self.normsq, max_norm, lr, momentum,
                          weight_decay)


class _FusedAttention(torch.autograd.Function):

    @staticmethod
    def forward(ctx, q, k, v, temperature):
        ext = require_native()
        q, k, v = q.contiguous(), k.contiguous(), v.contiguous()
        if q.size(1) <= 64:
            out, p = ext.attn_fwd(q, k, v, temperature)
            ctx.save_for_backward(q, k, v, p)
            ctx.blockwise = False
        else:
            out, lse = ext.attn_fwd_block(q, k, v, temperature)
            ctx.save_for_backward(q, k, v, out, lse)
            ctx.blockwise = True
        ctx.temperature = temperature
        return out

    @staticmethod
    def backward(ctx, dout):
        ext = require_native()
        if ctx.blockwise:
            q, k, v, out, lse = ctx.saved_tensors
            dq, dk, dv = ext.attn_bwd_block(dout, q, k, v, out, lse,
                                            ctx.temperature)
        else:
            q, k, v, p = ctx.saved_tensors
            dq, dk, dv = ext.attn_bwd(dout, q, k, v, p, ctx.temperature)
        return dq, dk, dv, None


def fused_attention(q, k, v, temperature):
    return _FusedAttention.apply(q, k, v, temperature)


class _FusedLayerNorm(torch.autograd.Function):

    @staticmethod
    def forward(ctx, x, weight, bias, R, eps):
        ext = require_native()
        x = x.contiguous()
        y, mean, invstd = ext.ln_fwd(x, weight, bias, R, eps)
        ctx.save_for_backward(x, weight, mean, invstd)
        ctx.R = R
        return y

    @staticmethod
    def backward(ctx, dy):
        ext = require_native()
        x, weight, mean, invstd = ctx.saved_tensors
        dx, dgamma, dbeta = ext.ln_bwd(dy, x, weight, mean, invstd, ctx.R)
        return dx, dgamma, dbeta, None, None


def fused_layernorm(x, weight, bias, R, eps=1e-5):
    return _FusedLayerNorm.apply(x, weight, bias, R, eps)


class _FusedLMCE(torch.autograd.Function):

    @staticmethod
    def forward(ctx, logits, tokens, mask, R):
        ext = require_native()
        logits = logits.contiguous()
        labels = tokens.reshape(-1)
        losses, _, row_max, row_logsum = ext.lm_ce_fwd(
            logits, labels, mask if mask is not None else torch.Tensor(), R)
        ctx.save_for_backward(logits, labels, row_max, row_logsum,
                              mask if mask is not None else torch.Tensor())
        ctx.R = R
        ctx.has_mask = mask is not None
        return losses

    @staticmethod
    def backward(ctx, up):
        ext = require_native()
        logits, labels, row_max, row_logsum, mask = ctx.saved_tensors
        d = ext.lm_ce_bwd(logits, labels,
                          mask if ctx.has_mask else torch.Tensor(), row_max,
                          row_logsum, up, ctx.R)
        return d, None, None, None


def fused_lm_ce(logits, tokens, mask, R):
    return _FusedLMCE.apply(logits, tokens, mask, R)


_rng_cells = {}
_rng_salt = [0]


def _next_salt():
    _rng_salt[0] = (_rng_salt[0] + 1) & 0x7FFFFFFF
    return _rng_salt[0]


def bump_rng(device):
    ext = require_native()
    ext.rng_bump(_rng_cell(device))


def _rng_cell(device):
    key = str(device)
    if key not in _rng_cells:
        _rng_cells[key] = torch.tensor(
            [torch.initial_seed() & 0x7FFFFFFFFFFFFFFF],
            dtype=torch.int64, device=device)
    return _rng_cells[key]


class _FusedGeluDropout(torch.autograd.Function):

    @staticmethod
    def forward(ctx, x, rate, p):
        ext = require_native()
        x = x.contiguous()
        y, mask = ext.gelu_drop_fwd(x, _rng_cell(x.device), _next_salt(),
                                    rate, p)
        ctx.save_for_backward(x, mask)
        ctx.meta = (rate, p)
        return y

    @staticmethod
    def backward(ctx, dy):
        ext = require_native()
        x, mask = ctx.saved_tensors
        rate, p = ctx.meta
        return ext.gelu_drop_bwd(dy, x, mask, rate, p), None, None


def fused_gelu_dropout(x, rate, p):
    return _FusedGeluDropout.apply(x, rate, p)


class _FusedResDropout(torch.autograd.Function):

    @staticmethod
    def forward(ctx, src, h, rate, p):
        ext = require_native()
        t, mask = ext.res_drop_fwd(src.contiguous(), h.contiguous(),
                                   _rng_cell(src.device), _next_salt(),
                                   rate, p)
        ctx.save_for_backward(mask)
        ctx.meta = (rate, p)
        return t

    @staticmethod
    def backward(ctx, dt):
        ext = require_native()
        (mask,) = ctx.saved_tensors
        rate, p = ctx.meta
        dh = ext.drop_scale_bwd(dt, mask, rate, p)
        return dt, dh, None, None


def fused_res_dropout(src, h, rate, p):
    return _FusedResDropout.apply(src, h, rate, p)


class _FusedScaler(torch.autograd.Function):

    @staticmethod
    def forward(ctx, x, rate):
        ext = require_native()
        ctx.rate = rate
        return ext.drop_scale_bwd(x.contiguous(), torch.Tensor(), rate, 0.0)

    @staticmethod
    def backward(ctx, dy):
        ext = require_native()
        return ext.drop_scale_bwd(dy.contiguous(), torch.Tensor(),
                                  ctx.rate, 0.0), None


def fused_scaler(x, rate):
    return _FusedScaler.apply(x, rate)


def fused_token_mask(tokens, rate, mask_id):
    ext = require_native()
    return ext.token_mask(tokens.contiguous(), _rng_cell(tokens.device),
                          _next_salt(), rate, mask_id)


class _FusedMaxPool2(torch.autograd.Function):

    @staticmethod
    def forward(ctx, x):
        ext = require_native()
        y, arg = ext.maxpool2_fwd(x.contiguous())
        ctx.save_for_backward(arg)
        ctx.hw = (x.size(2), x.size(3))
        return y

    @staticmethod
    def backward(ctx, dy):
        ext = require_native()
        (arg,) = ctx.saved_tensors
        return ext.maxpool2_bwd(dy, arg, *ctx.hw)


def fused_maxpool2(x):
    return _FusedMaxPool2.apply(x)


class _FusedEmbedPos(torch.autograd.Function):

    @staticmethod
    def forward(ctx, ids, table, pos, t16, p16, rate):
        ext = require_native()
        use16 = t16 is not None and p16 is not None
        t = t16 if use16 else table
        p = p16 if use16 else pos
        out = ext.embed_pos_fwd(ids.contiguous(), t.contiguous(),
                                p.contiguous(), rate)
        ctx.save_for_backward(ids)
        ctx.meta = (table.size(1), pos.size(1), rate)
        return out

    @staticmethod
    def backward(ctx, dy):
        ext = require_native()
        (ids,) = ctx.saved_tensors
        V, P, rate = ctx.meta
        dtable, dpos = ext.embed_pos_bwd(dy, ids, V, P, rate)
        return None, dtable, dpos, None, None, None


def fused_embed_pos(ids, table, pos, t16, p16, rate):
    return _FusedEmbedPos.apply(ids, table, pos, t16, p16, rate)


COMBINE_PER_BLOCK = 1024
_COMBINE_BLOCKS = {}


def _check_window(win, size, what):
    period, shift, take = win
    if not (period >= 1 and size % period == 0 and 0 <= shift < period
            and 1 <= take <= period):
        raise ValueError('combine_accumulate: bad {} window {} over an axis '
                         'of {}'.format(what, win, size))
    return (size // period) * take


def combine_accumulate(shapes, clients, device):
    import numpy as np
    ext = require_native()
    if ext is None:
        raise RuntimeError('combine_accumulate is the native route; use '
                           'Federation.accumulate under HETEROFL_FORCE_EAGER')
    device = torch.device(device)
    t_dt = np.dtype([('tmp', 'u8'), ('cnt', 'u8'), ('O', 'i4'), ('I', 'i4'),
                     ('inner', 'i4'), ('ent_start', 'i4'),
                     ('ent_count', 'i4'), ('pad', 'i4')])
    e_dt = np.dtype([('val', 'u8'), ('mask', 'u8'), ('out', 'i4', 3),
                     ('inp', 'i4', 3), ('n_in', 'i4'), ('pad', 'i4')])
    assert t_dt.itemsize == 40 and e_dt.itemsize == 48
    dims, numels = [], []
    for shape in shapes:
        shape = tuple(int(s) for s in shape)
        if len(shape) == 0:
            shape = (1,)
        O = shape[0]
        I = shape[1] if len(shape) > 1 else 1
        inner = 1
        for s in shape[2:]:
            inner *= s
        if O * I * inner >= 2 ** 31:
            raise ValueError('combine_accumulate: tensor too large')
        dims.append((O, I, inner))
        numels.append(O * I * inner)
    total = sum(numels)
    flat_tmp = torch.empty(total, dtype=torch.float32, device=device)
    flat_cnt = torch.empty(total, dtype=torch.float32, device=device)
    tensors = np.zeros(len(dims), dtype=t_dt)
    n_entries = sum(len(c) for c in clients)
    entries = np.zeros(n_entries, dtype=e_dt)
    masks, mask_off, keep = [], 0, []
    mask_rel = np.full(n_entries, -1, dtype=np.int64)
    e = off = 0
    tmp_out, cnt_out = [], []
    for i, ((O, I, inner), shape) in enumerate(zip(dims, shapes)):
        tmp = flat_tmp[off:off + numels[i]].view(tuple(shape))
        cnt = flat_cnt[off:off + numels[i]].view(tuple(shape))
        tmp_out.append(tmp)
        cnt_out.append(cnt)
        tensors[i] = (tmp.data_ptr(), cnt.data_ptr(), O, I, inner, e,
                      len(clients[i]), 0)
        off += numels[i]
        for val, ow, iw, mask in clients[i]:
            if iw is None:
                iw = (I, 0, I)
            n_out = _check_window(ow, O, 'out')
            n_in = _check_window(iw, I, 'in')
            if not (val.dtype == torch.float32 and val.device == device):
                raise ValueError('combine_accumulate: client values must be '
                                 'fp32 on {}'.format(device))
            if val.numel() != n_out * n_in * inner:
                raise ValueError(
                    'combine_accumulate: client slice of {} elements does '
                    'not match its windows ({} x {} x {})'.format(
                        val.numel(), n_out, n_in, inner))
            val = val.contiguous()
            keep.append(val)
            if mask is not None:
                mask = np.ascontiguousarray(mask, dtype=np.uint8).reshape(-1)
                if mask.size != n_out:
                    raise ValueError('combine_accumulate: row mask of {} '
                                     'for {} rows'.format(mask.size, n_out))
                mask_rel[e] = mask_off
                masks.append(mask)
                mask_off += mask.size
            entries[e] = (val.data_ptr(), 0, tuple(ow), tuple(iw), n_in, 0)
            e += 1
    bkey = (str(device), tuple(dims))
    blocks = _COMBINE_BLOCKS.get(bkey)
    if blocks is None:
        rows = [np.stack([np.full((n + COMBINE_PER_BLOCK - 1)
                                  // COMBINE_PER_BLOCK, i, dtype=np.int32),
                          np.arange(0, n, COMBINE_PER_BLOCK,
                                    dtype=np.int32)], 1)
                for i, n in enumerate(numels) if n]
        tab = np.concatenate(rows) if rows else np.zeros((0, 2), np.int32)
        if len(_COMBINE_BLOCKS) >= 16:
            _COMBINE_BLOCKS.clear()
        blocks = _COMBINE_BLOCKS[bkey] = \
            torch.from_numpy(np.ascontiguousarray(tab)).to(device)
    mask_base = tensors.nbytes + entries.nbytes
    table = torch.empty(mask_base + mask_off, dtype=torch.uint8,
                        device=device)
    has = mask_rel >= 0
    entries['mask'][has] = (table.data_ptr() + mask_base
                            + mask_rel[has]).astype(np.uint64)
    host = np.concatenate([tensors.view(np.uint8), entries.view(np.uint8)]
                          + masks)
    table.copy_(torch.from_numpy(host))
    ext.combine_accumulate(table, len(dims), n_entries, blocks)
    del keep
    return tmp_out, cnt_out
```

Before: 29480 samples/s.

## Fuse head+masked-CE, residual add into BN backward, and batch gather with counter

Adds a fused avgpool+per-client linear+masked cross-entropy kernel (forward and backward in one launch each), a BN+ReLU autograd op that returns the input as an alias so the identity-shortcut gradient is added inside the BN backward store, and a batch-gather kernel that copies the current batch and advances the step counter in one launch. All three cut kernel launches and intermediate tensors inside the captured training step, where small per-step kernels dominate at batch size 10. In exchange it adds new kernels with a grid-wide ticket counter and more code paths to keep consistent with the fallback.

```diff
diff --git a/heterofl_amd/fed/batched.py b/heterofl_amd/fed/batched.py
--- a/heterofl_amd/fed/batched.py
+++ b/heterofl_amd/fed/batched.py
@@ -130,6 +130,14 @@
         return eager_scaler_norm_relu(x, self.weight, self.bias, kind,
                                       self.groups, r)
 
+    def forward_alias(self, x):
+        if (self.norm == 'bn' and self.stats_sink is None
+                and native_ops.use_native(x) and native_ops.step_fused_on()
+                and torch.is_grad_enabled() and x.requires_grad):
+            from ..ops.fused import fused_norm_relu_alias
+            return fused_norm_relu_alias(x, self.weight, self.bias)
+        return self.forward(x), x
+
 
 class BMaxPool2(nn.Module):
 
@@ -168,8 +176,11 @@
                                     1, stride, 0, bias=False)
 
     def forward(self, x):
-        out = self.n1(x)
-        shortcut = self.shortcut(out) if hasattr(self, 'shortcut') else x
+        if hasattr(self, 'shortcut'):
+            out = self.n1(x)
+            shortcut = self.shortcut(out)
+        else:
+            out, shortcut = self.n1.forward_alias(x)
         out = self.conv1(out)
         return self.conv2(self.n2(out), residual=shortcut)
 
@@ -191,8 +202,11 @@
                                     1, stride, 0, bias=False)
 
     def forward(self, x):
-        out = self.n1(x)
-        shortcut = self.shortcut(out) if hasattr(self, 'shortcut') else x
+        if hasattr(self, 'shortcut'):
+            out = self.n1(x)
+            shortcut = self.shortcut(out)
+        else:
+            out, shortcut = self.n1.forward_alias(x)
         out = self.conv1(out)
         out = self.conv2(self.n2(out))
         return self.conv3(self.n3(out), residual=shortcut)
@@ -223,13 +237,19 @@
             self.in_planes = planes * block.expansion
         return nn.Sequential(*layers)
 
-    def forward(self, x):
+    def features(self, x):
         out = self.conv1(x)
         out = self.layer1(out)
         out = self.layer2(out)
         out = self.layer3(out)
         out = self.layer4(out)
-        out = self.n4(out)
+        return self.n4(out)
+
+    def head_params(self):
+        return self.linear.weight, self.linear.bias
+
+    def forward(self, x):
+        out = self.features(x)
         if native_ops.use_native(out):
             from ..ops.fused import fused_head
             return fused_head(out, self.linear.weight, self.linear.bias,
@@ -259,8 +279,14 @@
         self._feat = hidden_size[-1]
         self.head = BLinear(R, hidden_size[-1], num_classes)
 
-    def forward(self, x):
-        out = self.blocks(x)
+    def features(self, x):
+        return self.blocks(x)
+
+    def head_params(self):
+        return self.head.weight, self.head.bias
+
+    def forward(self, x):
+        out = self.features(x)
         if native_ops.use_native(out):
             from ..ops.fused import fused_head
             return fused_head(out, self.head.weight, self.head.bias, self.R)
@@ -340,6 +366,39 @@
             metrics[:, 1] += correct
             metrics[:, 2] += N
     return losses
+
+
+def step_losses(model, xb, yb, label_masks, metrics=None, amp=False,
+                fused=None):
+    if fused is None:
+        fused = native_ops.use_native(xb) and native_ops.step_fused_on()
+    dev = 'cuda' if xb.is_cuda else 'cpu'
+    if fused:
+        from ..ops.fused import fused_head_ce
+        with torch.autocast(dev, torch.bfloat16, enabled=amp):
+            feat = model.features(xb)
+        w, b = model.head_params()
+        return fused_head_ce(feat, w, b, yb, label_masks, model.R,
+                             metrics=metrics)
+    with torch.autocast(dev, torch.bfloat16, enabled=amp):
+        scores = model(xb)
+    losses = batched_masked_ce(scores.float(), yb, label_masks,
+                               metrics=metrics)
+    return losses, scores
+
+
+def step_grads(losses, params=None, fused=None, ones=None):
+    if fused is None:
+        fused = native_ops.use_native(losses) and native_ops.step_fused_on()
+    if not fused:
+        if params is None:
+            return losses.sum().backward()
+        return torch.autograd.grad(losses.sum(), params)
+    if ones is None:
+        ones = torch.ones_like(losses)
+    if params is None:
+        return torch.autograd.backward(losses, ones)
+    return torch.autograd.grad(losses, params, grad_outputs=ones)
 
 
 def per_client_clip_(params, R, max_norm=1.0):
@@ -604,10 +663,17 @@
                     torch._foreach_zero_([p.grad for p in params])
                 else:
                     opt.zero_grad(set_to_none=True)
-                with torch.autocast('cuda', torch.bfloat16, enabled=self._amp):
-                    scores = model(xb)
-                losses = batched_masked_ce(scores.float(), yb, masks)
-                losses.sum().backward()
+                if native:
+                    fused = native_ops.step_fused_on()
+                    losses, scores = step_losses(model, xb, yb, masks,
+                                                 amp=self._amp, fused=fused)
+                    step_grads(losses, fused=fused)
+                else:
+                    with torch.autocast('cuda', torch.bfloat16,
+                                        enabled=self._amp):
+                        scores = model(xb)
+                    losses = batched_masked_ce(scores.float(), yb, masks)
+                    losses.sum().backward()
                 if native:
                     fopt.step(1.0, lr, cfg['momentum'], cfg['weight_decay'])
                 else:
diff --git a/heterofl_amd/fed/graphs.py b/heterofl_amd/fed/graphs.py
--- a/heterofl_amd/fed/graphs.py
+++ b/heterofl_amd/fed/graphs.py
@@ -1,7 +1,7 @@
 import torch
 
 from .. import ops as native_ops
-from .batched import batched_masked_ce
+from .batched import batched_masked_ce, step_grads, step_losses
 
 
 class GraphedGroupStep:
@@ -25,6 +25,8 @@
         self.y_all = torch.zeros(capacity, R, dtype=torch.long, device=device)
         self.masks = torch.ones(R, classes, device=device)
         self.counter = torch.zeros(1, dtype=torch.long, device=device)
+        self._ticket = torch.zeros(1, dtype=torch.int32, device=device)
+        self._ones = torch.ones(R, device=device)
         self.metrics = torch.zeros(R, 3, device=device)
         self.graph = None
         self._arange = torch.arange(batch, device=device)
@@ -45,22 +47,29 @@
         return (self.R * in_ch, hw, hw)
 
     def _one_step(self):
-        idx = self.counter * self.batch + self._arange
-        xb = self.x_all.index_select(0, idx)
-        yb = self.y_all.index_select(0, idx)
-        if self._native:
-            with torch.autocast('cuda', torch.bfloat16, enabled=self.amp):
-                scores = self.model(xb)
-            losses = batched_masked_ce(scores.float(), yb, self.masks,
-                                       metrics=self.metrics)
-            raw = torch.autograd.grad(losses.sum(), self.params)
+        fused = self._native and native_ops.step_fused_on()
+        if fused:
+            from ..ops.fused import batch_gather
+            xb, yb = batch_gather(self.x_all, self.y_all, self.counter,
+                                  self.batch, self._ticket)
+        else:
+            idx = self.counter * self.batch + self._arange
+            xb = self.x_all.index_select(0, idx)
+            yb = self.y_all.index_select(0, idx)
+        if self._native:
+            losses, _ = step_losses(self.model, xb, yb, self.masks,
+                                    metrics=self.metrics, amp=self.amp,
+                                    fused=fused)
+            raw = step_grads(losses, self.params, fused=fused,
+                             ones=self._ones)
             grads = [t if t.is_contiguous() else t.contiguous() for t in raw]
             self._captured_grads = grads
             if not self._capturing:
                 self.opt.bind(grads)
             self.opt.launch(1.0, self.lr, self.momentum, self.weight_decay)
-            with torch.no_grad():
-                self.counter += 1
+            if not fused:
+                with torch.no_grad():
+                    self.counter += 1
             return
         with torch.autocast('cuda', torch.bfloat16, enabled=self.amp):
             scores = self.model(xb)
diff --git a/heterofl_amd/ops/__init__.py b/heterofl_amd/ops/__init__.py
--- a/heterofl_amd/ops/__init__.py
+++ b/heterofl_amd/ops/__init__.py
@@ -50,6 +50,13 @@
     return os.environ.get('HETEROFL_NATIVE_CONV', '1') == '1'
 
 
+def step_fused_on():
+    ext = _load()
+    if ext is not None:
+        return ext.step_fused_on()
+    return os.environ.get('HETEROFL_STEP_FUSED', '1')[:1] != '0'
+
+
 _FP8 = False
 
 
diff --git a/heterofl_amd/ops/csrc/batch_gather.hip b/heterofl_amd/ops/csrc/batch_gather.hip
--- /dev/null
+++ b/heterofl_amd/ops/csrc/batch_gather.hip
@@ -0,0 +1,101 @@
+#include "common.h"
+
+template <typename U>
+__device__ __forceinline__ void copy_units(const void* src, void* dst,
+                                           long units) {
+    const U* s = (const U*)src;
+    U* d = (U*)dst;
+    for (long i = (long)blockIdx.x * blockDim.x + threadIdx.x; i < units;
+         i += (long)gridDim.x * blockDim.x)
+        d[i] = s[i];
+}
+
+template <typename U>
+__device__ __forceinline__ void zero_units(void* dst, long units) {
+    U* d = (U*)dst;
+    for (long i = (long)blockIdx.x * blockDim.x + threadIdx.x; i < units;
+         i += (long)gridDim.x * blockDim.x)
+        d[i] = U{};
+}
+
+template <int XU>
+__global__ void __launch_bounds__(256)
+batch_gather_kernel(const char* __restrict__ x_all, const char* __restrict__ y_all,
+                    char* __restrict__ xb, char* __restrict__ yb,
+                    long* __restrict__ counter, unsigned* __restrict__ ticket,
+                    long last, long B, long x_row_bytes, long y_row_bytes) {
+    const long cnt = counter[0];
+    if (cnt >= 0 && cnt <= last) {
+        const long row0 = cnt * B;
+        const char* xs = x_all + row0 * x_row_bytes;
+        const long xbytes = B * x_row_bytes;
+        if (XU == 16) copy_units<uint4>(xs, xb, xbytes / 16);
+        else if (XU == 8) copy_units<unsigned long>(xs, xb, xbytes / 8);
+        else if (XU == 4) copy_units<unsigned>(xs, xb, xbytes / 4);
+        else if (XU == 2) copy_units<unsigned short>(xs, xb, xbytes / 2);
+        else copy_units<unsigned char>(xs, xb, xbytes);
+        copy_units<unsigned long>(y_all + row0 * y_row_bytes, yb,
+                                  B * y_row_bytes / 8);
+    } else {
+        zero_units<unsigned char>(xb, B * x_row_bytes);
+        zero_units<unsigned long>(yb, B * y_row_bytes / 8);
+    }
+    __syncthreads();
+    if (threadIdx.x == 0) {
+        __threadfence();
+        const unsigned t = atomicAdd(ticket, 1u);
+        if (t == gridDim.x - 1) {
+            counter[0] = cnt + 1;
+            atomicExch(ticket, 0u);
+        }
+    }
+}
+
+#include <torch/extension.h>
+#include <ATen/hip/HIPContext.h>
+
+std::vector<at::Tensor> batch_gather(at::Tensor x_all, at::Tensor y_all,
+                                     at::Tensor counter, at::Tensor ticket,
+                                     int64_t B) {
+    TORCH_CHECK(x_all.is_cuda() && x_all.is_contiguous() &&
+                y_all.is_cuda() && y_all.is_contiguous());
+    TORCH_CHECK(y_all.scalar_type() == at::kLong && y_all.dim() == 2);
+    TORCH_CHECK(counter.is_cuda() && counter.scalar_type() == at::kLong &&
+                counter.numel() == 1);
+    TORCH_CHECK(ticket.is_cuda() && ticket.scalar_type() == at::kInt &&
+                ticket.numel() == 1);
+    const long cap = x_all.size(0);
+    TORCH_CHECK(B >= 1 && B <= cap && y_all.size(0) == cap,
+                "batch_gather: batch / capacity mismatch");
+    auto xs = x_all.sizes().vec();
+    xs[0] = B;
+    auto xb = at::empty(xs, x_all.options());
+    auto yb = at::empty({(long)B, y_all.size(1)}, y_all.options());
+    const long esz = x_all.element_size();
+    const long x_row_bytes = x_all.numel() / cap * esz;
+    const long y_row_bytes = y_all.size(1) * 8;
+    const bool vec = x_row_bytes % 16 == 0 &&
+                     ptr_aligned(x_all.data_ptr(), 16) &&
+                     ptr_aligned(xb.data_ptr(), 16);
+    const int xu = vec ? 16 : (int)esz;
+    const long units = std::max(B * x_row_bytes / xu, B * y_row_bytes / 8);
+    const int grid = (int)std::min<long>(128, std::max<long>(1, (units + 255) / 256));
+    auto stream = at::hip::getCurrentHIPStream();
+#define LAUNCH_BG(XU)                                                         \
+    hipLaunchKernelGGL(batch_gather_kernel<XU>, dim3(grid), dim3(256), 0,     \
+                       stream, (const char*)x_all.data_ptr(),                 \
+                       (const char*)y_all.data_ptr(), (char*)xb.data_ptr(),   \
+                       (char*)yb.data_ptr(), (long*)counter.data_ptr(),       \
+                       (unsigned*)ticket.data_ptr(), cap / B - 1, (long)B,    \
+                       x_row_bytes, y_row_bytes)
+    switch (xu) {
+        case 16: LAUNCH_BG(16); break;
+        case 8: LAUNCH_BG(8); break;
+        case 4: LAUNCH_BG(4); break;
+        case 2: LAUNCH_BG(2); break;
+        case 1: LAUNCH_BG(1); break;
+        default: TORCH_CHECK(false, "batch_gather: unsupported element size");
+    }
+#undef LAUNCH_BG
+    return {xb, yb};
+}
diff --git a/heterofl_amd/ops/csrc/bindings.cpp b/heterofl_amd/ops/csrc/bindings.cpp
--- a/heterofl_amd/ops/csrc/bindings.cpp
+++ b/heterofl_amd/ops/csrc/bindings.cpp
@@ -115,6 +115,25 @@
                                      at::Tensor vocab_mask, int64_t V,
                                      int64_t E, int64_t k, int64_t splits);
 int64_t lm_head_topk_splits(int64_t M, int64_t V);
+std::vector<at::Tensor> bn_relu_bwd_add(at::Tensor dy, at::Tensor x,
+                                        at::Tensor gamma, at::Tensor beta,
+                                        at::Tensor mean, at::Tensor invstd,
+                                        at::Tensor addend);
+std::vector<at::Tensor> head_ce_fwd(at::Tensor feat, at::Tensor w,
+                                    at::Tensor b, at::Tensor labels,
+                                    at::Tensor mask, at::Tensor metrics,
+                                    int64_t R);
+std::vector<at::Tensor> head_ce_bwd(at::Tensor up, at::Tensor scores,
+                                    at::Tensor labels, at::Tensor mask,
+                                    at::Tensor pooled, at::Tensor w,
+                                    int64_t R, int64_t H, int64_t W,
+                                    bool bf16_feat, bool want_db);
+std::string head_ce_route(int64_t N, int64_t R, int64_t C, int64_t HW,
+                          int64_t J, int64_t elem_size, bool aligned);
+bool step_fused_on();
+std::vector<at::Tensor> batch_gather(at::Tensor x_all, at::Tensor y_all,
+                                     at::Tensor counter, at::Tensor ticket,
+                                     int64_t B);
 
 PYBIND11_MODULE(TORCH_EXTENSION_NAME, m) {
     m.def("bn_relu_fwd", &bn_relu_fwd, "fused sBN+ReLU forward");
@@ -144,6 +163,21 @@
     m.def("mfma_probe", &mfma_probe, "16x16x32 bf16 MFMA layout probe");
     m.def("head_fwd", &head_fwd, "fused avgpool+per-client-linear forward");
     m.def("head_bwd", &head_bwd, "fused head backward");
+    m.def("bn_relu_bwd_add", &bn_relu_bwd_add,
+          "fused sBN+ReLU backward with dx + addend in the dx store");
+    m.def("head_ce_fwd", &head_ce_fwd,
+          "avgpool + per-client linear + masked CE (+ metrics) forward, one "
+          "launch");
+    m.def("head_ce_bwd", &head_ce_bwd,
+          "masked CE backward + head backward, one launch");
+    m.def("head_ce_route", &head_ce_route,
+          "route head_ce_fwd / head_ce_bwd would take (vec / elem / chain); "
+          "launches nothing");
+    m.def("step_fused_on", &step_fused_on,
+          "HETEROFL_STEP_FUSED as the launchers read it");
+    m.def("batch_gather", &batch_gather,
+          "copy batch `counter` of the epoch buffers and advance the counter, "
+          "one launch");
     m.def("attn_fwd", &attn_fwd, "fused small-S attention forward");
     m.def("attn_bwd", &attn_bwd, "fused small-S attention backward");
     m.def("attn_fwd_block", &attn_fwd_block,
diff --git a/heterofl_amd/ops/csrc/fused_norm.hip b/heterofl_amd/ops/csrc/fused_norm.hip
--- a/heterofl_amd/ops/csrc/fused_norm.hip
+++ b/heterofl_amd/ops/csrc/fused_norm.hip
@@ -117,11 +117,23 @@
     }
 }
 
-template <typename T, bool STAGE>
+template <typename T>
+__device__ __forceinline__ float round_T(float v) {
+    T t;
+    st_f32(&t, v);
+    return ld_f32(&t);
+}
+__device__ __forceinline__ float add_rn(float a, float b) {
+#pragma clang fp contract(off)
+    return a + b;
+}
+
+template <typename T, bool STAGE, bool ADD>
 __global__ void __launch_bounds__(256)
 bn_relu_bwd_kernel(const T* __restrict__ dy, const T* __restrict__ x,
                    const float* __restrict__ gamma, const float* __restrict__ beta,
                    const float* __restrict__ mean, const float* __restrict__ invstd,
+                   const T* __restrict__ addend,
                    T* __restrict__ dx, float* __restrict__ dgamma,
                    float* __restrict__ dbeta, int N, int C, int HW) {
     const int c = blockIdx.x;
@@ -169,7 +181,11 @@
             const float pre = xh * g + b;
             d = pre > 0.f ? ld_f32(dy + off) : 0.f;
         }
-        st_f32(dx + off, gis * (d - k1 - xh * k2));
+        const float v = gis * (d - k1 - xh * k2);
+        if (ADD)
+            st_f32(dx + off, add_rn(round_T<T>(v), ld_f32(addend + off)));
+        else
+            st_f32(dx + off, v);
     }
 }
 
@@ -259,13 +275,14 @@
     }
 }
 
-template <typename T>
+template <typename T, bool ADD>
 __global__ void __launch_bounds__(256)
 bn_relu_bwd_vec_kernel(const T* __restrict__ dy, const T* __restrict__ x,
                        const float* __restrict__ gamma,
                        const float* __restrict__ beta,
                        const float* __restrict__ mean,
-                       const float* __restrict__ invstd, T* __restrict__ dx,
+                       const float* __restrict__ invstd,
+                       const T* __restrict__ addend, T* __restrict__ dx,
                        float* __restrict__ dgamma, float* __restrict__ dbeta,
                        int N, int C, int HW) {
     constexpr int V = 16 / sizeof(T);
@@ -282,6 +299,7 @@
     const T* xc = x + (long)c * HW;
     const T* dyc = dy + (long)c * HW;
     T* dxc = dx + (long)c * HW;
+    const T* adc = ADD ? addend + (long)c * HW : nullptr;
     const float m = mean[c], is = invstd[c];
     const float g = gamma ? gamma[c] : 1.f;
     const float b = beta ? beta[c] : 0.f;
@@ -333,6 +351,13 @@
             const float pre = xh * g + b;
             const float d = pre > 0.f ? fd[e] : 0.f;
             fd[e] = gis * (d - k1 - xh * k2);
+        }
+        if (ADD) {
+            float fa[V];
+            unpack16<T>(*(const uint4*)(adc + ww.n * samp_stride + ww.j * V),
+                        fa);
+#pragma unroll
+            for (int e = 0; e < V; ++e) fd[e] = add_rn(round_T<T>(fd[e]), fa[e]);
         }
         *(uint4*)(dxc + ww.n * samp_stride + ww.j * V) = pack16<T>(fd);
         ww.step();
@@ -534,9 +559,13 @@
     return {y, mean, invstd};
 }
 
-std::vector<at::Tensor> bn_relu_bwd(at::Tensor dy, at::Tensor x,
-                                    at::Tensor gamma, at::Tensor beta,
-                                    at::Tensor mean, at::Tensor invstd) {
+template <bool ADD>
+static std::vector<at::Tensor> bn_relu_bwd_impl(at::Tensor dy, at::Tensor x,
+                                                at::Tensor gamma,
+                                                at::Tensor beta,
+                                                at::Tensor mean,
+                                                at::Tensor invstd,
+                                                at::Tensor addend) {
     const int N = x.size(0), C = x.size(1);
     const int HW = x.numel() / (N * C);
     auto dx = at::empty_like(x);
@@ -544,27 +573,52 @@
     auto dgamma = at::empty({C}, opts);
     auto dbeta = at::empty({C}, opts);
     auto dyc = dy.contiguous();
+    at::Tensor adc;
+    if (ADD) {
+        TORCH_CHECK(addend.is_cuda() && addend.sizes() == x.sizes() &&
+                        addend.scalar_type() == x.scalar_type(),
+                    "bn_relu_bwd_add: addend must match x");
+        adc = addend.contiguous();
+    }
     auto stream = at::hip::getCurrentHIPStream();
     const long stage_bytes = 2L * N * (x.numel() / (N * C)) * x.element_size();
     const BnRoute route = bn_route(true, N, HW, (int)x.element_size(),
                                    ptr_aligned(x.data_ptr(), 16) &&
                                        ptr_aligned(dyc.data_ptr(), 16) &&
-                                       ptr_aligned(dx.data_ptr(), 16));
+                                       ptr_aligned(dx.data_ptr(), 16) &&
+                                       (!ADD ||
+                                        ptr_aligned(adc.data_ptr(), 16)));
     const float* gp = gamma.defined() ? gamma.data_ptr<float>() : nullptr;
     const float* bp = beta.defined() ? beta.data_ptr<float>() : nullptr;
     DISPATCH_FT(x.scalar_type(), {
-        auto kern = route == BN_VEC ? bn_relu_bwd_vec_kernel<scalar_t>
-                    : route == BN_STAGED ? bn_relu_bwd_kernel<scalar_t, true>
-                                         : bn_relu_bwd_kernel<scalar_t, false>;
+        auto kern = route == BN_VEC ? bn_relu_bwd_vec_kernel<scalar_t, ADD>
+                    : route == BN_STAGED
+                        ? bn_relu_bwd_kernel<scalar_t, true, ADD>
+                        : bn_relu_bwd_kernel<scalar_t, false, ADD>;
         hipLaunchKernelGGL(kern, dim3(C), dim3(256),
                            route == BN_DIRECT ? 0 : (int)stage_bytes, stream,
                            (const scalar_t*)dyc.data_ptr(),
                            (const scalar_t*)x.data_ptr(), gp, bp,
                            mean.data_ptr<float>(), invstd.data_ptr<float>(),
+                           ADD ? (const scalar_t*)adc.data_ptr() : nullptr,
                            (scalar_t*)dx.data_ptr(), dgamma.data_ptr<float>(),
                            dbeta.data_ptr<float>(), N, C, HW);
     });
     return {dx, dgamma, dbeta};
+}
+
+std::vector<at::Tensor> bn_relu_bwd(at::Tensor dy, at::Tensor x,
+                                    at::Tensor gamma, at::Tensor beta,
+                                    at::Tensor mean, at::Tensor invstd) {
+    return bn_relu_bwd_impl<false>(dy, x, gamma, beta, mean, invstd,
+                                   at::Tensor());
+}
+
+std::vector<at::Tensor> bn_relu_bwd_add(at::Tensor dy, at::Tensor x,
+                                        at::Tensor gamma, at::Tensor beta,
+                                        at::Tensor mean, at::Tensor invstd,
+                                        at::Tensor addend) {
+    return bn_relu_bwd_impl<true>(dy, x, gamma, beta, mean, invstd, addend);
 }
 
 std::vector<at::Tensor> gn_relu_fwd(at::Tensor x, at::Tensor gamma,
diff --git a/heterofl_amd/ops/csrc/head_ce.hip b/heterofl_amd/ops/csrc/head_ce.hip
--- /dev/null
+++ b/heterofl_amd/ops/csrc/head_ce.hip
@@ -0,0 +1,356 @@
+#include "common.h"
+
+constexpr int HCE_FWD_THREADS = 1024;
+constexpr int HCE_CS = 32;
+constexpr long HCE_LDS = 64 * 1024;
+
+template <typename T, bool VEC>
+__global__ void __launch_bounds__(HCE_FWD_THREADS)
+head_ce_fwd_kernel(const T* __restrict__ feat, const float* __restrict__ w,
+                   const float* __restrict__ b,
+                   const long* __restrict__ labels,
+                   const float* __restrict__ mask, float* __restrict__ pooled,
+                   float* __restrict__ scores, float* __restrict__ losses,
+                   float* __restrict__ metrics, int N, int R, int C, int HW,
+                   int J) {
+    const int r = blockIdx.x;
+    const int CP = C + 1;
+    extern __shared__ float lds[];
+    float* sp = lds;
+    float* sw = sp + N * CP;
+    float* ss = sw + J * CP;
+    const float* wr0 = w + (long)r * J * C;
+    for (int e = threadIdx.x; e < J * C; e += blockDim.x) {
+        const int j = e / C, c = e - j * C;
+        sw[j * CP + c] = wr0[e];
+    }
+    const float inv_hw = 1.f / HW;
+    for (int e = threadIdx.x; e < N * C; e += blockDim.x) {
+        const int n = e / C, c = e - n * C;
+        const T* src = feat + ((long)n * R * C + (long)r * C + c) * HW;
+        float s = 0.f;
+        if (VEC) {
+            constexpr int V = 16 / sizeof(T);
+            const uint4* src4 = (const uint4*)src;
+            for (int v = 0; v < HW / V; ++v) {
+                float f[V];
+                unpack16<T>(src4[v], f);
+#pragma unroll
+                for (int k = 0; k < V; ++k) s += f[k];
+            }
+        } else {
+            for (int i = 0; i < HW; ++i) s += ld_f32(src + i);
+        }
+        const float m = s * inv_hw;
+        sp[n * CP + c] = m;
+        pooled[((long)n * R + r) * C + c] = m;
+    }
+    __syncthreads();
+    for (int e = threadIdx.x; e < N * J; e += blockDim.x) {
+        const int n = e / J, j = e - n * J;
+        const float* wr = sw + j * CP;
+        const float* pr = sp + n * CP;
+        float s = b ? b[r * J + j] : 0.f;
+        for (int c = 0; c < C; ++c) s = __fmaf_rn(pr[c], wr[c], s);
+        ss[e] = s;
+        scores[((long)n * R + r) * J + j] = s;
+    }
+    __syncthreads();
+    if (threadIdx.x >= WAVE) return;
+    const int lane = threadIdx.x;
+    float loss = 0.f;
+    int correct = 0;
+    for (int n = lane; n < N; n += WAVE) {
+        const float* s = ss + n * J;
+        const long y = labels[(long)n * R + r];
+        float mx = -1e30f;
+        int arg = 0;
+        for (int c = 0; c < J; ++c) {
+            float v = s[c];
+            if (mask) v = mask[r * J + c] != 0.f ? v : 0.f;
+            if (v > mx) { mx = v; arg = c; }
+        }
+        float lse = 0.f;
+        for (int c = 0; c < J; ++c) {
+            float v = s[c];
+            if (mask) v = mask[r * J + c] != 0.f ? v : 0.f;
+            lse += __expf(v - mx);
+        }
+        lse = mx + __logf(lse);
+        float vy = s[y];
+        if (mask) vy = mask[r * J + y] != 0.f ? vy : 0.f;
+        loss += lse - vy;
+        correct += (arg == y);
+    }
+    for (int off = WAVE / 2; off > 0; off >>= 1) {
+        loss += __shfl_down(loss, off, WAVE);
+        correct += __shfl_down(correct, off, WAVE);
+    }
+    if (lane == 0) {
+        losses[r] = loss / N;
+        if (metrics) {
+            metrics[r * 3 + 0] += loss;
+            metrics[r * 3 + 1] += correct;
+            metrics[r * 3 + 2] += N;
+        }
+    }
+}
+
+template <typename T, bool VEC>
+__global__ void __launch_bounds__(256)
+head_ce_bwd_kernel(const float* __restrict__ up, long up_stride,
+                   const float* __restrict__ scores,
+                   const long* __restrict__ labels,
+                   const float* __restrict__ mask,
+                   const float* __restrict__ pooled,
+                   const float* __restrict__ w, float* __restrict__ dw,
+                   float* __restrict__ db, T* __restrict__ dfeat, int N,
+                   int R, int C, int HW, int J) {
+    const int r = blockIdx.x;
+    const int c0 = blockIdx.y * HCE_CS;
+    const int cs = min(HCE_CS, C - c0);
+    extern __shared__ float lds[];
+    float* ds = lds;
+    float* sw = ds + N * J;
+    for (int e = threadIdx.x; e < J * cs; e += blockDim.x) {
+        const int j = e / cs, c = e - j * cs;
+        sw[j * HCE_CS + c] = w[((long)r * J + j) * C + c0 + c];
+    }
+    for (int n = threadIdx.x; n < N; n += blockDim.x) {
+        const long i = (long)n * R + r;
+        const float* s = scores + i * J;
+        float* dsr = ds + n * J;
+        const long y = labels[i];
+        float mx = -1e30f;
+        for (int c = 0; c < J; ++c) {
+            float v = s[c];
+            if (mask) v = mask[r * J + c] != 0.f ? v : 0.f;
+            mx = fmaxf(mx, v);
+        }
+        float denom = 0.f;
+        for (int c = 0; c < J; ++c) {
+            float v = s[c];
+            if (mask) v = mask[r * J + c] != 0.f ? v : 0.f;
+            denom += __expf(v - mx);
+        }
+        const float scale = up[r * up_stride] / N;
+        for (int c = 0; c < J; ++c) {
+            float v = s[c];
+            bool live = true;
+            if (mask) live = mask[r * J + c] != 0.f;
+            v = live ? v : 0.f;
+            float g = __expf(v - mx) / denom - (c == y ? 1.f : 0.f);
+            dsr[c] = live ? scale * g : 0.f;
+        }
+    }
+    __syncthreads();
+    for (int e = threadIdx.x; e < J * cs; e += blockDim.x) {
+        const int j = e / cs, c = c0 + e - j * cs;
+        float s = 0.f;
+        for (int n = 0; n < N; ++n)
+            s = __fmaf_rn(ds[n * J + j], pooled[((long)n * R + r) * C + c], s);
+        dw[((long)r * J + j) * C + c] = s;
+    }
+    if (db && blockIdx.y == 0) {
+        for (int j = threadIdx.x; j < J; j += blockDim.x) {
+            float s = 0.f;
+            for (int n = 0; n < N; ++n) s += ds[n * J + j];
+            db[r * J + j] = s;
+        }
+    }
+    const float inv_hw = 1.f / HW;
+    for (int e = threadIdx.x; e < N * cs; e += blockDim.x) {
+        const int n = e / cs, c = e - n * cs;
+        float s = 0.f;
+        for (int j = 0; j < J; ++j)
+            s = __fmaf_rn(ds[n * J + j], sw[j * HCE_CS + c], s);
+        const float g = s * inv_hw;
+        T* dst = dfeat + ((long)n * R * C + (long)r * C + c0 + c) * HW;
+        if (VEC) {
+            constexpr int V = 16 / sizeof(T);
+            float f[V];
+#pragma unroll
+            for (int k = 0; k < V; ++k) f[k] = g;
+            const uint4 q = pack16<T>(f);
+            uint4* dst4 = (uint4*)dst;
+            for (int v = 0; v < HW / V; ++v) dst4[v] = q;
+        } else {
+            for (int i = 0; i < HW; ++i) st_f32(dst + i, g);
+        }
+    }
+}
+
+#include <torch/extension.h>
+#include <ATen/hip/HIPContext.h>
+
+std::vector<at::Tensor> head_fwd(at::Tensor feat, at::Tensor w, at::Tensor b,
+                                 int64_t R);
+std::vector<at::Tensor> head_bwd(at::Tensor dscores, at::Tensor pooled,
+                                 at::Tensor w, int64_t R, int64_t H,
+                                 int64_t W, bool bf16_feat, bool want_db);
+std::vector<at::Tensor> masked_ce_fwd(at::Tensor scores, at::Tensor labels,
+                                      at::Tensor mask, at::Tensor metrics);
+at::Tensor masked_ce_bwd(at::Tensor scores, at::Tensor labels, at::Tensor mask,
+                         at::Tensor up);
+
+bool step_fused_on() {
+    const char* e = std::getenv("HETEROFL_STEP_FUSED");
+    return !(e && e[0] == '0');
+}
+
+enum HceRoute { HCE_VEC, HCE_ELEM, HCE_CHAIN };
+
+static bool present(const at::Tensor& t) {
+    return t.defined() && t.numel() > 0;
+}
+
+static HceRoute hce_route(long N, long C, long HW, long J, int esz,
+                          bool aligned) {
+    if (!step_fused_on()) return HCE_CHAIN;
+    if (N < 1 || C < 1 || J < 1 || HW < 1) return HCE_CHAIN;
+    const long fwd = ((N + J) * (C + 1) + N * J) * 4;
+    const long bwd = (N * J + J * HCE_CS) * 4;
+    if (fwd > HCE_LDS || bwd > HCE_LDS) return HCE_CHAIN;
+    return aligned && (HW * esz) % 16 == 0 ? HCE_VEC : HCE_ELEM;
+}
+
+std::string head_ce_route(int64_t N, int64_t R, int64_t C, int64_t HW,
+                          int64_t J, int64_t elem_size, bool aligned) {
+    (void)R;
+    static const char* names[] = {"vec", "elem", "chain"};
+    return names[hce_route(N, C, HW, J, (int)elem_size, aligned)];
+}
+
+#define DISPATCH_HCE(t, vec, ...)                                             \
+    if ((t) == at::kFloat) {                                                  \
+        using scalar_t = float;                                               \
+        if (vec) { constexpr bool kVec = true; __VA_ARGS__; }                 \
+        else { constexpr bool kVec = false; __VA_ARGS__; }                    \
+    } else if ((t) == at::kBFloat16) {                                        \
+        using scalar_t = __hip_bfloat16;                                      \
+        if (vec) { constexpr bool kVec = true; __VA_ARGS__; }                 \
+        else { constexpr bool kVec = false; __VA_ARGS__; }                    \
+    } else { TORCH_CHECK(false, "unsupported dtype"); }
+
+std::vector<at::Tensor> head_ce_fwd(at::Tensor feat, at::Tensor w,
+                                    at::Tensor b, at::Tensor labels,
+                                    at::Tensor mask, at::Tensor metrics,
+                                    int64_t R) {
+    TORCH_CHECK(feat.is_cuda() && feat.is_contiguous() && w.is_contiguous());
+    TORCH_CHECK(labels.is_contiguous() && labels.scalar_type() == at::kLong);
+    TORCH_CHECK(w.scalar_type() == at::kFloat);
+    const int N = feat.size(0);
+    const int C = (int)(feat.size(1) / R);
+    const int HW = feat.numel() / std::max<int64_t>(1, N * feat.size(1));
+    const int J = w.size(1);
+    const HceRoute route = hce_route(N, C, HW, J, (int)feat.element_size(),
+                                     ptr_aligned(feat.data_ptr(), 16));
+    if (route == HCE_CHAIN) {
+        auto sp = head_fwd(feat, w, b, R);
+        auto l = masked_ce_fwd(sp[0], labels, mask, metrics);
+        return {l[0], sp[1], sp[0]};
+    }
+    TORCH_CHECK(R >= 1 && feat.dim() == 4 && feat.size(1) == R * C,
+                "head_ce_fwd: feat channels must be R * C");
+    TORCH_CHECK(w.is_cuda() && w.dim() == 3 && w.size(0) == R &&
+                    w.size(2) == C,
+                "head_ce_fwd: w must be (R, J, C) on the device");
+    TORCH_CHECK(labels.is_cuda() && labels.dim() == 2 &&
+                    labels.size(0) == N && labels.size(1) == R,
+                "head_ce_fwd: labels must be (N, R) on the device");
+    TORCH_CHECK(!present(mask) || (mask.is_cuda() && mask.is_contiguous() &&
+                                   mask.scalar_type() == at::kFloat &&
+                                   mask.numel() == R * J),
+                "head_ce_fwd: mask must be (R, J) fp32 on the device");
+    TORCH_CHECK(!present(b) || (b.is_cuda() && b.is_contiguous() &&
+                                b.scalar_type() == at::kFloat &&
+                                b.numel() == R * J),
+                "head_ce_fwd: b must be (R, J) fp32 on the device");
+    TORCH_CHECK(!present(metrics) || (metrics.is_cuda() &&
+                                      metrics.is_contiguous() &&
+                                      metrics.scalar_type() == at::kFloat &&
+                                      metrics.numel() == R * 3),
+                "head_ce_fwd: metrics must be (R, 3) fp32 on the device");
+    auto opts = feat.options().dtype(at::kFloat);
+    auto pooled = at::empty({N, (long)R, C}, opts);
+    auto scores = at::empty({N, (long)R, J}, opts);
+    auto losses = at::empty({(long)R}, opts);
+    auto stream = at::hip::getCurrentHIPStream();
+    const int lds = (int)(((long)(N + J) * (C + 1) + (long)N * J) * 4);
+    DISPATCH_HCE(feat.scalar_type(), route == HCE_VEC, {
+        hipLaunchKernelGGL((head_ce_fwd_kernel<scalar_t, kVec>),
+                           dim3((int)R), dim3(HCE_FWD_THREADS), lds, stream,
+                           (const scalar_t*)feat.data_ptr(),
+                           w.data_ptr<float>(),
+                           present(b) ? b.data_ptr<float>() : nullptr,
+                           labels.data_ptr<long>(),
+                           present(mask) ? mask.data_ptr<float>() : nullptr,
+                           pooled.data_ptr<float>(), scores.data_ptr<float>(),
+                           losses.data_ptr<float>(),
+                           present(metrics) ? metrics.data_ptr<float>()
+                                             : nullptr,
+                           N, (int)R, C, HW, J);
+    });
+    return {losses, pooled, scores};
+}
+
+std::vector<at::Tensor> head_ce_bwd(at::Tensor up, at::Tensor scores,
+                                    at::Tensor labels, at::Tensor mask,
+                                    at::Tensor pooled, at::Tensor w,
+                                    int64_t R, int64_t H, int64_t W,
+                                    bool bf16_feat, bool want_db) {
+    const auto feat_dtype = bf16_feat ? at::kBFloat16 : at::kFloat;
+    const int N = scores.size(0);
+    const int J = scores.size(2);
+    const int C = pooled.size(2);
+    const int HW = (int)(H * W);
+    const int esz = bf16_feat ? 2 : 4;
+    HceRoute route = hce_route(N, C, HW, J, esz, true);
+    if (route == HCE_CHAIN || up.scalar_type() != at::kFloat ||
+        up.dim() != 1) {
+        auto dsc = masked_ce_bwd(scores, labels, mask, up);
+        return head_bwd(dsc, pooled, w, R, H, W, bf16_feat, want_db);
+    }
+    TORCH_CHECK(scores.is_cuda() && scores.is_contiguous() &&
+                    scores.scalar_type() == at::kFloat && scores.dim() == 3 &&
+                    scores.size(1) == R,
+                "head_ce_bwd: scores must be (N, R, J) fp32 on the device");
+    TORCH_CHECK(pooled.is_cuda() && pooled.is_contiguous() &&
+                    pooled.scalar_type() == at::kFloat && pooled.dim() == 3 &&
+                    pooled.size(0) == N && pooled.size(1) == R,
+                "head_ce_bwd: pooled must be (N, R, C) fp32 on the device");
+    TORCH_CHECK(w.is_cuda() && w.is_contiguous() &&
+                    w.scalar_type() == at::kFloat && w.dim() == 3 &&
+                    w.size(0) == R && w.size(1) == J && w.size(2) == C,
+                "head_ce_bwd: w must be (R, J, C) fp32 on the device");
+    TORCH_CHECK(labels.is_cuda() && labels.is_contiguous() &&
+                    labels.scalar_type() == at::kLong &&
+                    labels.numel() == (long)N * R,
+                "head_ce_bwd: labels must be (N, R) int64 on the device");
+    TORCH_CHECK(!present(mask) || (mask.is_cuda() && mask.is_contiguous() &&
+                                   mask.scalar_type() == at::kFloat &&
+                                   mask.numel() == R * J),
+                "head_ce_bwd: mask must be (R, J) fp32 on the device");
+    TORCH_CHECK(up.is_cuda() && up.size(0) == R,
+                "head_ce_bwd: up must be (R,) on the device");
+    auto opts = pooled.options();
+    auto dw = at::empty({(long)R, J, C}, opts);
+    auto db = want_db ? at::empty({(long)R, J}, opts) : at::Tensor();
+    auto dfeat = at::empty({N, (long)R * C, H, W}, opts.dtype(feat_dtype));
+    if (!ptr_aligned(dfeat.data_ptr(), 16)) route = HCE_ELEM;
+    auto stream = at::hip::getCurrentHIPStream();
+    const int lds = (int)(((long)N * J + (long)J * HCE_CS) * 4);
+    const dim3 grid((int)R, (C + HCE_CS - 1) / HCE_CS);
+    DISPATCH_HCE(feat_dtype, route == HCE_VEC, {
+        hipLaunchKernelGGL((head_ce_bwd_kernel<scalar_t, kVec>), grid,
+                           dim3(256), lds, stream, up.data_ptr<float>(),
+                           (long)up.stride(0), scores.data_ptr<float>(),
+                           labels.data_ptr<long>(),
+                           present(mask) ? mask.data_ptr<float>() : nullptr,
+                           pooled.data_ptr<float>(), w.data_ptr<float>(),
+                           dw.data_ptr<float>(),
+                           want_db ? db.data_ptr<float>() : nullptr,
+                           (scalar_t*)dfeat.data_ptr(), N, (int)R, C, HW, J);
+    });
+    return {dw, db, dfeat};
+}
diff --git a/heterofl_amd/ops/fused.py b/heterofl_amd/ops/fused.py
--- a/heterofl_amd/ops/fused.py
+++ b/heterofl_amd/ops/fused.py
@@ -34,6 +34,59 @@
 
 def fused_norm_relu(x, weight, bias, kind, groups=1, eps=1e-5):
     return _FusedNormReLU.apply(x, weight, bias, kind, groups, eps)
+
+
+class _FusedNormReLUAlias(torch.autograd.Function):
+
+    @staticmethod
+    def forward(ctx, x, weight, bias, eps):
+        ctx.set_materialize_grads(False)
+        ctx.native = use_native(x)
+        if ctx.native:
+            ext = require_native()
+            xc = x.contiguous()
+            y, mean, invstd = ext.bn_relu_fwd(xc, weight, bias, eps)
+        else:
+            xc = x
+            mean = x.mean(dim=(0, 2, 3))
+            var = x.var(dim=(0, 2, 3), unbiased=False)
+            invstd = (var + eps).rsqrt()
+            cv = (1, -1, 1, 1)
+            y = F.relu((x - mean.view(cv)) * (invstd * weight).view(cv)
+                       + bias.view(cv))
+        ctx.save_for_backward(xc, weight, bias, mean, invstd)
+        return y, x
+
+    @staticmethod
+    def backward(ctx, dy, dalias):
+        x, weight, bias, mean, invstd = ctx.saved_tensors
+        if dy is None:
+            dy = torch.zeros_like(x)
+        if ctx.native:
+            ext = require_native()
+            if dalias is None:
+                dx, dgamma, dbeta = ext.bn_relu_bwd(dy, x, weight, bias, mean,
+                                                    invstd)
+            else:
+                dx, dgamma, dbeta = ext.bn_relu_bwd_add(
+                    dy, x, weight, bias, mean, invstd, dalias.to(x.dtype))
+            return dx, dgamma, dbeta, None
+        cv = (1, -1, 1, 1)
+        M = x.numel() // x.size(1)
+        xh = (x - mean.view(cv)) * invstd.view(cv)
+        pre = xh * weight.view(cv) + bias.view(cv)
+        d = torch.where(pre > 0, dy, torch.zeros_like(dy))
+        dbeta = d.sum((0, 2, 3))
+        dgamma = (d * xh).sum((0, 2, 3))
+        dx = (weight * invstd).view(cv) * (d - (dbeta / M).view(cv)
+                                           - xh * (dgamma / M).view(cv))
+        if dalias is not None:
+            dx = dx + dalias
+        return dx, dgamma, dbeta, None
+
+
+def fused_norm_relu_alias(x, weight, bias, eps=1e-5):
+    return _FusedNormReLUAlias.apply(x, weight, bias, eps)
 
 
 def bn_relu_route(direction, N, C, HW, elem_size, aligned=True):
@@ -363,6 +416,63 @@
 
 def fused_head(feat, weight, bias, R):
     return _FusedHead.apply(feat, weight, bias, R)
+
+
+class _FusedHeadCE(torch.autograd.Function):
+
+    @staticmethod
+    def forward(ctx, feat, weight, bias, labels, mask, metrics, R):
+        ext = require_native()
+        feat = feat.contiguous()
+        none = torch.Tensor()
+        labels = labels.contiguous()
+        losses, pooled, scores = ext.head_ce_fwd(
+            feat, weight, bias if bias is not None else none, labels,
+            mask if mask is not None else none,
+            metrics if metrics is not None else none, R)
+        ctx.save_for_backward(scores, labels,
+                              mask if mask is not None else none, pooled,
+                              weight)
+        ctx.meta = (R, feat.size(2), feat.size(3),
+                    feat.dtype == torch.bfloat16, bias is not None,
+                    mask is not None)
+        ctx.mark_non_differentiable(scores)
+        return losses, scores
+
+    @staticmethod
+    def backward(ctx, up, _dscores):
+        ext = require_native()
+        scores, labels, mask, pooled, weight = ctx.saved_tensors
+        R, H, W, bf16_feat, has_bias, has_mask = ctx.meta
+        dw, db, dfeat = ext.head_ce_bwd(
+            up, scores, labels, mask if has_mask else torch.Tensor(), pooled,
+            weight, R, H, W, bf16_feat, has_bias)
+        return (dfeat, dw, (db if has_bias else None), None, None, None,
+                None)
+
+
+def fused_head_ce(feat, weight, bias, labels, mask, R, metrics=None):
+    if use_native(feat):
+        return _FusedHeadCE.apply(feat, weight, bias, labels, mask, metrics,
+                                  R)
+    from ..fed.batched import batched_masked_ce
+    pooled = F.adaptive_avg_pool2d(feat, 1).view(feat.size(0), R, -1)
+    scores = torch.einsum('nri,roi->nro', pooled, weight)
+    if bias is not None:
+        scores = scores + bias
+    losses = batched_masked_ce(scores.float(), labels, mask, metrics=metrics)
+    return losses, scores
+
+
+def head_ce_route(N, R, C, HW, J, elem_size, aligned=True):
+    ext = require_native()
+    return ext.head_ce_route(N, R, C, HW, J, elem_size, aligned)
+
+
+def batch_gather(x_all, y_all, counter, B, ticket):
+    ext = require_native()
+    xb, yb = ext.batch_gather(x_all, y_all, counter, ticket, B)
+    return xb, yb
 
 
 class GraphClipSGD:
```

Result: faster. 30660 samples/s (median of 6 runs) (+4.0%).
